# chenxing1999/recsys-benchmark

Hardware: NVIDIA B200
Metric: DeepFM train samples/s (Criteo shape) (higher is better)
Workload: dtype f32

## Files before the change

include/rsb.h:

```cpp
#ifndef RSB_H_
#define RSB_H_

#include <stdint.h>

#if defined(__GNUC__)
#define RSB_API __attribute__((visibility("default")))
#else
#define RSB_API
#endif

#ifdef __cplusplus
extern "C" {
#endif

typedef enum {
  RSB_OK = 0,
  RSB_ERR_BAD_ARG = 10001,
  RSB_ERR_UNSUPPORTED = 10002,
  RSB_ERR_WORKSPACE = 10003
} rsb_status;

typedef enum {
  RSB_KIND_VANILLA = 0,
  RSB_KIND_QR_MULT = 1,
  RSB_KIND_QR_ADD = 2,
  RSB_KIND_QR_CAT = 3,
  RSB_KIND_PEP = 4,
  RSB_KIND_MASK = 5,
  RSB_KIND_OPTEMBED = 6
} rsb_kind;

typedef enum {
  RSB_PEP_GLOBAL = 0,
  RSB_PEP_DIMENSION = 1,
  RSB_PEP_FEATURE = 2,
  RSB_PEP_FEATURE_DIM = 3
} rsb_pep_threshold;

typedef enum {
  RSB_APPLY_DENSE = 0,
  RSB_APPLY_SPARSE_ADAM = 1,
  RSB_APPLY_SPARSE_SGD = 2,
  RSB_APPLY_SHARD_ATOMIC = 3
} rsb_apply;

RSB_API const char* rsb_version(void);
RSB_API const char* rsb_error_string(int code);
RSB_API int64_t rsb_launch_count(void);
RSB_API int rsb_row_width_supported(int32_t width);

RSB_API int rsb_lookup_fwd(int32_t kind, const void* idx, int32_t idx_is_i32, const int64_t* offsets,
                   int64_t B, int32_t F, int32_t D,
                   const float* table, int64_t n_rows, int64_t n_global,
                   const float* table1, int64_t divider,
                   const void* aux, int32_t aux_mode, const int64_t* mask_d_idx,
                   const float* fc, const float* bias,
                   float* out_emb, float* out_yfm, float* out_sum, int64_t* out_rows,
                   int32_t* err_flag, float* amax_slots, void* stream);
#define RSB_LOOKUP_AMAX_SLOTS 1024

RSB_API int rsb_lookup_bwd_rows(int32_t kind, const int64_t* rows, int64_t B, int32_t F, int32_t D,
                        const float* table, int64_t n_rows, const float* table1, int64_t divider,
                        const void* aux, int32_t aux_mode, const int64_t* mask_d_idx,
                        const float* emb, const float* S, const float* g_yfm, const float* g_deep,
                        float* rg_main, float* rg_aux, float* fc_grad, void* stream);

RSB_API int rsb_fc_grad(const int64_t* rows, const float* g_yfm, int64_t B, int32_t F, float* fc_grad, void* stream);

RSB_API int rsb_fc_grad_sorted(const uint32_t* sorted_keys, const uint32_t* perm, int64_t n, const float* g_yfm, int32_t F,
                               float* fc_grad, void* workspace, int64_t workspace_bytes, void* stream);

RSB_API int64_t rsb_qr_bwd_fused_workspace_bytes(int64_t B, int32_t D);
RSB_API int rsb_qr_bwd_fused(int32_t kind, const int64_t* rows, int64_t B, int32_t F, int32_t D,
                             const float* table, int64_t n_rows, const float* table1, int64_t divider,
                             const float* emb, const float* S, const float* g_yfm, const float* g_deep,
                             float* rg_main, float* table1_grad, float* fc_grad, void* workspace,
                             int64_t workspace_bytes, void* stream);

RSB_API int64_t rsb_sort_workspace_bytes(int64_t n);
RSB_API int rsb_sort_rows(const int64_t* keys, int64_t n, int64_t n_rows, int64_t key_div, int64_t key_mod,
                  uint32_t* sorted_keys, uint32_t* perm, void* workspace, int64_t workspace_bytes,
                  void* stream);

RSB_API int64_t rsb_segment_workspace_bytes(int64_t n, int32_t E);
RSB_API int rsb_segment_reduce_apply(int32_t apply, const uint32_t* sorted_keys, const uint32_t* perm, int64_t n,
                             const float* row_grads, int32_t E,
                             float* dst, float* exp_avg, float* exp_avg_sq,
                             float lr, float beta1, float beta2, float eps, int64_t step,
                             void* workspace, int64_t workspace_bytes, void* stream);

RSB_API int64_t rsb_small_table_workspace_bytes(int64_t n_rows, int32_t E);
RSB_API int rsb_small_table_grad(const int64_t* keys, int64_t n, int64_t key_div, int64_t key_mod,
                         const float* row_grads, int32_t E, int64_t n_rows, float* dst,
                         void* workspace, int64_t workspace_bytes, void* stream);

RSB_API int rsb_pep_threshold_table(const float* weight, const float* s, int32_t threshold_type, int64_t n_rows,
                            int32_t D, float* out, int64_t* count, void* stream);
RSB_API int rsb_pep_dense_bwd(const float* weight, const float* s, int32_t threshold_type, int64_t n_rows, int32_t D,
                      const float* g_table, float* g_weight, float* g_s_full, void* stream);
RSB_API int rsb_optembed_eval_weight(const float* weight, const float* t_row, const int64_t* mask_d_row, int32_t norm,
                             int64_t n_rows, int32_t D, float* out, int64_t* count, void* stream);
RSB_API int rsb_mask_table(const float* weight, const uint8_t* mask, int64_t numel, float* out, void* stream);
RSB_API int rsb_sigmoid(const float* s, int64_t numel, float* out, void* stream);

RSB_API int rsb_csr_lookup_fwd(const void* idx, int32_t idx_is_i32, const int64_t* offsets, int64_t B, int32_t F,
                               int32_t D, const float* values, const void* crow, int32_t crow_bytes, const void* col,
                               int32_t col_bytes, int64_t n_rows, const float* fc, const float* bias, float* out_emb,
                               float* out_yfm, int32_t* err_flag, void* stream);

RSB_API int rsb_dhe_encode(const void* ids, int32_t ids_is_i32, int64_t n, int64_t prefix, const int64_t* slopes,
                           const int64_t* bias, const int64_t* primes, int32_t k, int64_t m, int32_t small_operands,
                           float* out, void* stream);

typedef enum { RSB_PLANES_BF16X3 = 0, RSB_PLANES_FP16X2 = 1 } rsb_planes_format_id;
typedef struct {
  int32_t format;
  int32_t max_scale_exp;
  float* amax;
} rsb_planes_format;

typedef struct {
  const void* planes;
  int64_t rows, cols, ld, plane_stride;
  int32_t mn_major;
  int64_t batch_row_step, batch_col_step;
  rsb_planes_format fmt;
} rsb_planes_operand;

typedef enum {
  RSB_EPI_LINEAR = 0,
  RSB_EPI_RELU_DROPOUT_PLANES = 1,
  RSB_EPI_MASK_PLANES = 2,
  RSB_EPI_MASK_F32 = 3
} rsb_epilogue_mode;

typedef struct {
  int32_t mode;
  void* out_planes;
  int64_t out_ld, out_plane_stride;
  int32_t ones_col;
  uint8_t* mask;
  float p;
  float* d_amax;
  float* bn_partials;
} rsb_gemm_epilogue;

RSB_API int rsb_relu_dropout_planes(const float* x, int64_t M, int32_t N, int64_t ldx, float p, uint64_t seed, uint64_t offset,
                                    const uint64_t* offset_dev, int32_t ones_col, void* out_planes, int64_t out_ld,
                                    int64_t plane_stride, uint8_t* mask, void* stream);
RSB_API int rsb_dropout_keep_mask(uint8_t* mask, int64_t numel, float p, uint64_t seed, uint64_t offset,
                                  const uint64_t* offset_dev, void* stream);

RSB_API int rsb_split_planes(const float* in, int64_t rows, int64_t cols, int64_t ld, int32_t transpose, int32_t ones_col,
                             void* out_planes, int64_t out_ld, int64_t plane_stride, const rsb_planes_format* fmt ,
                             void* stream);
RSB_API int rsb_rank1_absmax(const float* g_row, int64_t M, const float* w_col, int64_t N, float mul, float* amax_out,
                             void* stream);
RSB_API int rsb_absmax(const float* in, int64_t rows, int64_t cols, int64_t ld, float* amax_out, void* stream);
RSB_API int rsb_rank1_mask_planes(const float* g_row, const float* w_col, const uint8_t* mask, int64_t M, int32_t N, float p,
                                  void* out_planes, int64_t out_ld, int64_t plane_stride, void* stream);
RSB_API int64_t rsb_gemm_planes_workspace_bytes(int64_t M, int64_t N, int64_t K, int64_t batch, int32_t split_k);
RSB_API int rsb_gemm_planes(const rsb_planes_operand* A, const rsb_planes_operand* B, int64_t M, int64_t N, int64_t K,
                            int64_t batch, int32_t split_k, const float* C, float* D, int64_t ldd, int64_t d_batch_stride,
                            const float* bias, float alpha, float beta, const rsb_gemm_epilogue* epilogue ,
                            void* workspace, int64_t workspace_bytes, void* stream);

RSB_API int64_t rsb_bn_workspace_bytes(int64_t M, int32_t N);
RSB_API int rsb_bn_train_fwd_stats(const float* z, int64_t M, int32_t N, int64_t ldz, const float* gamma, const float* beta,
                                   float eps, float momentum, float* running_mean, float* running_var, float* stats,
                                   float* affine, float bound_mul, float* act_amax, void* workspace, int64_t workspace_bytes,
                                   void* stream);
RSB_API int64_t rsb_gemm_bn_partials_bytes(int64_t M, int64_t N, int64_t K, int32_t format);
RSB_API int rsb_bn_finalize_partials(const float* parts, int64_t M, int32_t N, const float* gamma, const float* beta, float eps,
                                     float momentum, float* running_mean, float* running_var, float* stats, float* affine,
                                     float bound_mul, float* act_amax, void* workspace, int64_t workspace_bytes, void* stream);
RSB_API int rsb_bn_relu_dropout_planes(const float* z, int64_t M, int32_t N, int64_t ldz, const float* affine, float p,
                                       uint64_t seed, uint64_t offset, const uint64_t* offset_dev, int32_t ones_col,
                                       void* out_planes, int64_t out_ld, int64_t plane_stride, uint8_t* mask,
                                       const rsb_planes_format* fmt , void* stream);
RSB_API int rsb_bn_train_bwd_planes(const float* g, const float* z, int64_t M, int32_t N, int64_t ldg, int64_t ldz,
                                    const float* stats, const float* gamma, float* sums, void* out_planes, int64_t out_ld,
                                    int64_t plane_stride, const rsb_planes_format* fmt ,
                                    const float* g_amax , void* workspace,
                                    int64_t workspace_bytes, void* stream);

RSB_API int rsb_relu_dropout_fwd(const float* x, int64_t numel, float p, uint64_t seed, uint64_t offset,
                                 const uint64_t* offset_dev , float* y,
                                 uint8_t* mask, void* stream);
RSB_API int rsb_relu_dropout_bwd(const float* g, const uint8_t* mask, int64_t M, int32_t N, float p, float* gx,
                                 float* colsum, void* workspace, int64_t workspace_bytes, void* stream);
RSB_API int64_t rsb_colsum_workspace_bytes(int64_t M, int32_t N);
RSB_API int rsb_colsum(const float* x, int64_t M, int32_t N, int64_t ld, float* out, void* workspace,
                       int64_t workspace_bytes, void* stream);
RSB_API int rsb_relu_dropout_dot_fwd(const float* x, int64_t M, int32_t N, float p, uint64_t seed, uint64_t offset,
                                     const uint64_t* offset_dev, const float* w, const float* bias, const float* affine,
                                     float* y, uint8_t* mask, float* out, void* stream);
RSB_API int rsb_relu_dropout_bwd_rank1(const float* g_row, const float* w_col, const uint8_t* mask, int64_t M, int32_t N,
                                       float p, float* gx, float* colsum, void* workspace, int64_t workspace_bytes,
                                       void* stream);
RSB_API int rsb_colsum_weighted(const float* x, const float* row_weight, int64_t M, int32_t N, int64_t ld, float* out,
                                void* workspace, int64_t workspace_bytes, void* stream);

RSB_API int rsb_dcn_gate_mix_fwd(const float* p2, const float* xl, const float* gates, int64_t B, int32_t Dm,
                                 int32_t E, int32_t r, float* h2, float* g, float* g2, void* stream);
RSB_API int rsb_dcn_cross_out_fwd(const float* t0, const float* x0, const float* xl, const float* bias,
                                  const float* g, int64_t B, int32_t Dm, int32_t E, float* x_next, void* stream);
RSB_API int rsb_dcn_cross_out_bwd(const float* g_next, const float* x0, const float* t0, const float* bias,
                                  const float* g, int64_t B, int32_t Dm, int32_t E, float* gT, float* gx0,
                                  float* dsg, void* stream);
RSB_API int rsb_dcn_gate_mix_bwd(const float* g_g2, const float* h2, const float* g, const float* dsg,
                                 const float* gates, const float* g_next, int64_t B, int32_t Dm, int32_t E,
                                 int32_t r, float* g_p2, float* dg, float* g_xl, void* stream);

#define RSB_IPC_HANDLE_BYTES 64
RSB_API int rsb_shared_alloc(int64_t bytes, void** dev_ptr_out );
RSB_API int rsb_shared_free(void* dev_ptr);
RSB_API int rsb_ipc_get_handle(const void* dev_ptr, uint8_t* h_handle );
RSB_API int rsb_ipc_open_handle(const uint8_t* h_handle , void** dev_ptr_out );
RSB_API int rsb_ipc_close_handle(void* dev_ptr);
RSB_API int rsb_lookup_fwd_sharded(const void* idx, int32_t idx_is_i32, const int64_t* offsets, int64_t B, int32_t F,
                                   int32_t D, const float* const* table_shards, const float* fc_replicated,
                                   int32_t G, int64_t n_global, const float* bias, const float* hot_table,
                                   const int64_t* hot_map, float* out_emb, float* out_yfm,
                                   float* out_sum, int64_t* out_rows, int32_t* err_flag, float* amax_slots ,
                                   void* stream);
RSB_API int rsb_lookup_fwd_sharded_kind(int32_t kind, const void* idx, int32_t idx_is_i32, const int64_t* offsets, int64_t B,
                                        int32_t F, int32_t D, const float* const* table_shards, int32_t G, int64_t n_rows,
                                        int64_t n_global, const float* table1, int64_t divider, const void* aux,
                                        const void* const* aux_shards, int32_t aux_mode, const int64_t* mask_d_idx,
                                        const float* fc_replicated, const float* bias, float* out_emb, float* out_yfm,
                                        float* out_sum, int64_t* out_rows, int32_t* err_flag, float* amax_slots, void* stream);
RSB_API int rsb_lookup_bwd_rows_sharded(int32_t kind, const int64_t* rows, int64_t B, int32_t F, int32_t D,
                                        const float* const* table_shards, int32_t G, int64_t n_rows, const float* table1,
                                        int64_t divider, const void* aux, const void* const* aux_shards, int32_t aux_mode,
                                        const int64_t* mask_d_idx, const float* emb, const float* S, const float* g_yfm,
                                        const float* g_deep, float* rg_main, float* rg_aux, void* stream);
RSB_API int rsb_segment_scatter_shards(const uint32_t* sorted_keys, const uint32_t* perm, int64_t n,
                                       const float* row_grads, int32_t E, float* const* grad_shards, int32_t G,
                                       float scale, const int64_t* hot_map, int32_t n_fields, float* hot_grad,
                                       void* workspace, int64_t workspace_bytes, void* stream);

RSB_API int rsb_records_unpack(const void* records, int64_t B, int32_t F, int32_t* ids_out, float* labels_out, void* stream);

#define RSB_ADAM_CHUNK 4096
#define RSB_ADAM_MAX_TENSORS 64
typedef struct {
  float* param;
  const float* grad;
  float* exp_avg;
  float* exp_avg_sq;
  int64_t numel;
} rsb_adam_tensor;
RSB_API int rsb_adam_dense(const rsb_adam_tensor* h_tensors, int32_t n_tensors, const int32_t* block_map, int64_t n_blocks,
                           double lr, double beta1, double beta2, double eps, double weight_decay, int64_t step, void* stream);

#ifdef __cplusplus
}
#endif
#endif
```

recsys-benchmark_b200/_lib.py:

```python
from __future__ import annotations

import ctypes as C
import os
from typing import Optional

import torch

_PKG = os.path.dirname(os.path.abspath(__file__))
LIB_PATH = os.path.join(_PKG, "librsb.so")

KIND_VANILLA, KIND_QR_MULT, KIND_QR_ADD, KIND_QR_CAT, KIND_PEP, KIND_MASK, KIND_OPTEMBED = range(7)
PEP_GLOBAL, PEP_DIMENSION, PEP_FEATURE, PEP_FEATURE_DIM = range(4)
APPLY_DENSE, APPLY_SPARSE_ADAM, APPLY_SPARSE_SGD, APPLY_SHARD_ATOMIC = range(4)

PEP_TYPES = {"global": PEP_GLOBAL, "dimension": PEP_DIMENSION, "feature": PEP_FEATURE,
             "feature_dim": PEP_FEATURE_DIM}
QR_KINDS = {"mult": KIND_QR_MULT, "add": KIND_QR_ADD, "cat": KIND_QR_CAT}

_p, _i32, _i64, _f = C.c_void_p, C.c_int32, C.c_int64, C.c_float

class PlanesFormat(C.Structure):

    _fields_ = [("format", C.c_int32), ("max_scale_exp", C.c_int32), ("amax", C.c_void_p)]


PLANES_BF16X3, PLANES_FP16X2 = 0, 1


class PlanesOperand(C.Structure):

    _fields_ = [("planes", C.c_void_p), ("rows", C.c_int64), ("cols", C.c_int64), ("ld", C.c_int64),
                ("plane_stride", C.c_int64), ("mn_major", C.c_int32), ("batch_row_step", C.c_int64),
                ("batch_col_step", C.c_int64), ("fmt", PlanesFormat)]


class GemmEpilogue(C.Structure):

    _fields_ = [("mode", C.c_int32), ("out_planes", C.c_void_p), ("out_ld", C.c_int64), ("out_plane_stride", C.c_int64),
                ("ones_col", C.c_int32), ("mask", C.c_void_p), ("p", C.c_float), ("d_amax", C.c_void_p),
                ("bn_partials", C.c_void_p)]


EPI_LINEAR, EPI_RELU_DROPOUT_PLANES, EPI_MASK_PLANES, EPI_MASK_F32 = range(4)

PROTOTYPES = {
    "rsb_version": (C.c_char_p, []),
    "rsb_error_string": (C.c_char_p, [C.c_int]),
    "rsb_launch_count": (_i64, []),
    "rsb_row_width_supported": (C.c_int, [_i32]),
    "rsb_lookup_fwd": (C.c_int, [_i32, _p, _i32, _p, _i64, _i32, _i32, _p, _i64, _i64, _p, _i64, _p, _i32, _p,
                                 _p, _p, _p, _p, _p, _p, _p, _p, _p]),
    "rsb_lookup_bwd_rows": (C.c_int, [_i32, _p, _i64, _i32, _i32, _p, _i64, _p, _i64, _p, _i32, _p, _p, _p, _p, _p,
                                      _p, _p, _p, _p]),
    "rsb_fc_grad": (C.c_int, [_p, _p, _i64, _i32, _p, _p]),
    "rsb_fc_grad_sorted": (C.c_int, [_p, _p, _i64, _p, _i32, _p, _p, _i64, _p]),
    "rsb_qr_bwd_fused_workspace_bytes": (_i64, [_i64, _i32]),
    "rsb_qr_bwd_fused": (C.c_int, [_i32, _p, _i64, _i32, _i32, _p, _i64, _p, _i64, _p, _p, _p, _p, _p, _p, _p, _p,
                                   _i64, _p]),
    "rsb_sort_workspace_bytes": (_i64, [_i64]),
    "rsb_sort_rows": (C.c_int, [_p, _i64, _i64, _i64, _i64, _p, _p, _p, _i64, _p]),
    "rsb_segment_workspace_bytes": (_i64, [_i64, _i32]),
    "rsb_segment_reduce_apply": (C.c_int, [_i32, _p, _p, _i64, _p, _i32, _p, _p, _p, _f, _f, _f, _f, _i64, _p,
                                           _i64, _p]),
    "rsb_small_table_workspace_bytes": (_i64, [_i64, _i32]),
    "rsb_small_table_grad": (C.c_int, [_p, _i64, _i64, _i64, _p, _i32, _i64, _p, _p, _i64, _p]),
    "rsb_pep_threshold_table": (C.c_int, [_p, _p, _i32, _i64, _i32, _p, _p, _p]),
    "rsb_pep_dense_bwd": (C.c_int, [_p, _p, _i32, _i64, _i32, _p, _p, _p, _p]),
    "rsb_optembed_eval_weight": (C.c_int, [_p, _p, _p, _i32, _i64, _i32, _p, _p, _p]),
    "rsb_mask_table": (C.c_int, [_p, _p, _i64, _p, _p]),
    "rsb_sigmoid": (C.c_int, [_p, _i64, _p, _p]),
    "rsb_csr_lookup_fwd": (C.c_int, [_p, _i32, _p, _i64, _i32, _i32, _p, _p, _i32, _p, _i32, _i64, _p, _p, _p, _p,
                                     _p, _p]),
    "rsb_dhe_encode": (C.c_int, [_p, _i32, _i64, _i64, _p, _p, _p, _i32, _i64, _i32, _p, _p]),
    "rsb_split_planes": (C.c_int, [_p, _i64, _i64, _i64, _i32, _i32, _p, _i64, _i64, C.POINTER(PlanesFormat), _p]),
    "rsb_absmax": (C.c_int, [_p, _i64, _i64, _i64, _p, _p]),
    "rsb_rank1_absmax": (C.c_int, [_p, _i64, _p, _i64, _f, _p, _p]),
    "rsb_relu_dropout_planes": (C.c_int, [_p, _i64, _i32, _i64, _f, C.c_uint64, C.c_uint64, _p, _i32, _p, _i64, _i64, _p, _p]),
    "rsb_dropout_keep_mask": (C.c_int, [_p, _i64, _f, C.c_uint64, C.c_uint64, _p, _p]),
    "rsb_rank1_mask_planes": (C.c_int, [_p, _p, _p, _i64, _i32, _f, _p, _i64, _i64, _p]),
    "rsb_gemm_planes_workspace_bytes": (_i64, [_i64, _i64, _i64, _i64, _i32]),
    "rsb_gemm_planes": (C.c_int, [C.POINTER(PlanesOperand), C.POINTER(PlanesOperand), _i64, _i64, _i64, _i64, _i32, _p,
                                  _p, _i64, _i64, _p, _f, _f, C.POINTER(GemmEpilogue), _p, _i64, _p]),
    "rsb_relu_dropout_fwd": (C.c_int, [_p, _i64, _f, C.c_uint64, C.c_uint64, _p, _p, _p, _p]),
    "rsb_relu_dropout_bwd": (C.c_int, [_p, _p, _i64, _i32, _f, _p, _p, _p, _i64, _p]),
    "rsb_colsum_workspace_bytes": (_i64, [_i64, _i32]),
    "rsb_colsum": (C.c_int, [_p, _i64, _i32, _i64, _p, _p, _i64, _p]),
    "rsb_relu_dropout_dot_fwd": (C.c_int, [_p, _i64, _i32, _f, C.c_uint64, C.c_uint64, _p, _p, _p, _p, _p, _p, _p, _p]),
    "rsb_bn_workspace_bytes": (_i64, [_i64, _i32]),
    "rsb_gemm_bn_partials_bytes": (_i64, [_i64, _i64, _i64, _i32]),
    "rsb_bn_finalize_partials": (C.c_int, [_p, _i64, _i32, _p, _p, _f, _f, _p, _p, _p, _p, _f, _p, _p, _i64, _p]),
    "rsb_bn_train_fwd_stats": (C.c_int, [_p, _i64, _i32, _i64, _p, _p, _f, _f, _p, _p, _p, _p, _f, _p, _p, _i64, _p]),
    "rsb_bn_relu_dropout_planes": (C.c_int, [_p, _i64, _i32, _i64, _p, _f, C.c_uint64, C.c_uint64, _p, _i32, _p, _i64, _i64,
                                             _p, C.POINTER(PlanesFormat), _p]),
    "rsb_bn_train_bwd_planes": (C.c_int, [_p, _p, _i64, _i32, _i64, _i64, _p, _p, _p, _p, _i64, _i64,
                                          C.POINTER(PlanesFormat), _p, _p, _i64, _p]),
    "rsb_relu_dropout_bwd_rank1": (C.c_int, [_p, _p, _p, _i64, _i32, _f, _p, _p, _p, _i64, _p]),
    "rsb_colsum_weighted": (C.c_int, [_p, _p, _i64, _i32, _i64, _p, _p, _i64, _p]),
    "rsb_dcn_gate_mix_fwd": (C.c_int, [_p, _p, _p, _i64, _i32, _i32, _i32, _p, _p, _p, _p]),
    "rsb_dcn_cross_out_fwd": (C.c_int, [_p, _p, _p, _p, _p, _i64, _i32, _i32, _p, _p]),
    "rsb_dcn_cross_out_bwd": (C.c_int, [_p, _p, _p, _p, _p, _i64, _i32, _i32, _p, _p, _p, _p]),
    "rsb_dcn_gate_mix_bwd": (C.c_int, [_p, _p, _p, _p, _p, _p, _i64, _i32, _i32, _i32, _p, _p, _p, _p]),
    "rsb_shared_alloc": (C.c_int, [_i64, C.POINTER(C.c_void_p)]),
    "rsb_shared_free": (C.c_int, [_p]),
    "rsb_ipc_get_handle": (C.c_int, [_p, C.c_char_p]),
    "rsb_ipc_open_handle": (C.c_int, [C.c_char_p, C.POINTER(C.c_void_p)]),
    "rsb_ipc_close_handle": (C.c_int, [_p]),
    "rsb_lookup_fwd_sharded": (C.c_int, [_p, _i32, _p, _i64, _i32, _i32, _p, _p, _i32, _i64, _p, _p, _p, _p, _p, _p,
                                         _p, _p, _p, _p]),
    "rsb_records_unpack": (C.c_int, [_p, _i64, _i32, _p, _p, _p]),
    "rsb_adam_dense": (C.c_int, [_p, _i32, _p, _i64, C.c_double, C.c_double, C.c_double, C.c_double, C.c_double, _i64, _p]),
    "rsb_lookup_fwd_sharded_kind": (C.c_int, [_i32, _p, _i32, _p, _i64, _i32, _i32, _p, _i32, _i64, _i64, _p, _i64, _p, _p,
                                              _i32, _p, _p, _p, _p, _p, _p, _p, _p, _p, _p]),
    "rsb_lookup_bwd_rows_sharded": (C.c_int, [_i32, _p, _i64, _i32, _i32, _p, _i32, _i64, _p, _i64, _p, _p, _i32, _p, _p,
                                              _p, _p, _p, _p, _p, _p]),
    "rsb_segment_scatter_shards": (C.c_int, [_p, _p, _i64, _p, _i32, _p, _i32, _f, _p, _i32, _p, _p, _i64, _p]),
}
LOOKUP_AMAX_SLOTS = 1024
ADAM_CHUNK = 4096
ADAM_MAX_TENSORS = 64


class AdamTensor(C.Structure):

    _fields_ = [("param", C.c_void_p), ("grad", C.c_void_p), ("exp_avg", C.c_void_p), ("exp_avg_sq", C.c_void_p),
                ("numel", C.c_int64)]

_lib: Optional[C.CDLL] = None


def load() -> C.CDLL:
    global _lib
    if _lib is not None:
        return _lib
    if not os.path.exists(LIB_PATH):
        raise RuntimeError(
            f"rsb: {LIB_PATH} not found. Build it with `python recsys-benchmark_b200/build.py` "
            "(or __graft_entry__.build()). There is no CPU / PyTorch fallback for the hot path.")
    lib = C.CDLL(LIB_PATH)
    for name, (res, args) in PROTOTYPES.items():
        fn = getattr(lib, name)
        fn.restype = res
        fn.argtypes = args
    _lib = lib
    return lib


def version() -> str:
    return load().rsb_version().decode()


def check(rc: int, what: str = "") -> None:
    if rc != 0:
        msg = load().rsb_error_string(int(rc)).decode()
        raise RuntimeError(f"rsb {what} failed (code {rc}): {msg}")


def ptr(t: Optional[torch.Tensor]) -> Optional[int]:
    if t is None:
        return None
    return t.data_ptr()


_raw_stream = getattr(torch._C, "_cuda_getCurrentRawStream", None)


def stream_ptr(device=None) -> int:
    if _raw_stream is not None and type(device) is torch.device and device.index is not None:
        return _raw_stream(device.index)
    return torch.cuda.current_stream(device).cuda_stream


def require_cuda(*tensors) -> torch.device:
    dev = None
    for t in tensors:
        if t is None:
            continue
        if not t.is_cuda:
            raise RuntimeError("rsb: the hot path runs on CUDA tensors only (no CPU fallback); "
                               "move the module and its inputs to a B200 device")
        if dev is None:
            dev = t.device
        elif t.device != dev:
            raise RuntimeError(f"rsb: tensors on different devices ({dev} vs {t.device})")
    return dev
```

recsys-benchmark_b200/csrc/batchnorm.cu:

```cuda
#include <cuda_bf16.h>

#include "common.cuh"

namespace rsb {

constexpr int kBnThreads = 128;

template <int MODE>
__global__ void __launch_bounds__(kBnThreads) bn_slab_sums_kernel(const float* __restrict__ z, const float* __restrict__ g,
                                                                  long long M, int N, long long ldz, long long ldg,
                                                                  const float* __restrict__ mean,
                                                                  const float* __restrict__ rstd,
                                                                  float* __restrict__ partials) {
  const int n4 = N / 4;
  const long long rows_per = (M + gridDim.x - 1) / gridDim.x;
  const long long r0 = rows_per * blockIdx.x;
  long long r1 = r0 + rows_per;
  if (r1 > M) r1 = M;
  for (int c4 = threadIdx.x; c4 < n4; c4 += kBnThreads) {
    float4 k, rs = make_float4(1.f, 1.f, 1.f, 1.f);
    if (MODE == 0) {
      k = __ldg(reinterpret_cast<const float4*>(z) + c4);
    } else {
      k = __ldg(reinterpret_cast<const float4*>(mean) + c4);
      rs = __ldg(reinterpret_cast<const float4*>(rstd) + c4);
    }
    float4 sa = make_float4(0.f, 0.f, 0.f, 0.f), sb = sa;
    long long r = r0;
    constexpr int U = MODE == 0 ? 8 : 4;
    for (; r + U <= r1; r += U) {
      float4 zv[U], gv[U];
#pragma unroll
      for (int u = 0; u < U; ++u) {
        zv[u] = __ldg(reinterpret_cast<const float4*>(z + (r + u) * ldz) + c4);
        if (MODE == 1) gv[u] = __ldg(reinterpret_cast<const float4*>(g + (r + u) * ldg) + c4);
      }
#pragma unroll
      for (int u = 0; u < U; ++u) {
        const float4 d = make_float4(zv[u].x - k.x, zv[u].y - k.y, zv[u].z - k.z, zv[u].w - k.w);
        if (MODE == 0) {
          sa.x += d.x; sa.y += d.y; sa.z += d.z; sa.w += d.w;
          sb.x = fmaf(d.x, d.x, sb.x); sb.y = fmaf(d.y, d.y, sb.y); sb.z = fmaf(d.z, d.z, sb.z); sb.w = fmaf(d.w, d.w, sb.w);
        } else {
          sa.x += gv[u].x; sa.y += gv[u].y; sa.z += gv[u].z; sa.w += gv[u].w;
          sb.x = fmaf(gv[u].x, d.x * rs.x, sb.x); sb.y = fmaf(gv[u].y, d.y * rs.y, sb.y);
          sb.z = fmaf(gv[u].z, d.z * rs.z, sb.z); sb.w = fmaf(gv[u].w, d.w * rs.w, sb.w);
        }
      }
    }
    for (; r < r1; ++r) {
      const float4 zv = __ldg(reinterpret_cast<const float4*>(z + r * ldz) + c4);
      const float4 d = make_float4(zv.x - k.x, zv.y - k.y, zv.z - k.z, zv.w - k.w);
      if (MODE == 0) {
        sa.x += d.x; sa.y += d.y; sa.z += d.z; sa.w += d.w;
        sb.x = fmaf(d.x, d.x, sb.x); sb.y = fmaf(d.y, d.y, sb.y); sb.z = fmaf(d.z, d.z, sb.z); sb.w = fmaf(d.w, d.w, sb.w);
      } else {
        const float4 gv = __ldg(reinterpret_cast<const float4*>(g + r * ldg) + c4);
        sa.x += gv.x; sa.y += gv.y; sa.z += gv.z; sa.w += gv.w;
        sb.x = fmaf(gv.x, d.x * rs.x, sb.x); sb.y = fmaf(gv.y, d.y * rs.y, sb.y);
        sb.z = fmaf(gv.z, d.z * rs.z, sb.z); sb.w = fmaf(gv.w, d.w * rs.w, sb.w);
      }
    }
    float* pa = partials + ((long long)blockIdx.x * 2) * N;
    reinterpret_cast<float4*>(pa)[c4] = sa;
    reinterpret_cast<float4*>(pa + N)[c4] = sb;
  }
}

template <int MODE>
__global__ void __launch_bounds__(1024) bn_finalize_kernel(const float* __restrict__ partials, int nblk, int N, long long M,
                                                          const float* __restrict__ z_row0, const float* __restrict__ gamma,
                                                          const float* __restrict__ beta, float eps, float momentum,
                                                          float* __restrict__ running_mean, float* __restrict__ running_var,
                                                          float* __restrict__ stats, float* __restrict__ affine,
                                                          const float* __restrict__ fwd_stats, float bound_mul,
                                                          const float* __restrict__ g_amax, float* __restrict__ amax) {
  __shared__ double red_a[32][33], red_b[32][33];
  const int tx = threadIdx.x & 31, ty = threadIdx.x >> 5;
  const int c = blockIdx.x * 32 + tx;
  float fa = 0.f, fb = 0.f, ca = 0.f, cb = 0.f;
  if (c < N) {
#pragma unroll 4
    for (int b = ty; b < nblk; b += 32) {
      const float va = __ldg(partials + ((long long)b * 2) * N + c) - ca;
      const float vb = __ldg(partials + ((long long)b * 2 + 1) * N + c) - cb;
      const float ta = __fadd_rn(fa, va), tb = __fadd_rn(fb, vb);
      ca = __fsub_rn(__fsub_rn(ta, fa), va);
      cb = __fsub_rn(__fsub_rn(tb, fb), vb);
      fa = ta;
      fb = tb;
    }
  }
  red_a[ty][tx] = (double)fa - (double)ca;
  red_b[ty][tx] = (double)fb - (double)cb;
  __syncthreads();
  if (ty != 0 || c >= N) return;
  double sa = 0.0, sb = 0.0;
#pragma unroll
  for (int y = 0; y < 32; ++y) {
    sa += red_a[y][tx];
    sb += red_b[y][tx];
  }
  if (MODE == 0) {
    const double m = (double)M;
    const double dm = sa / m;
    double var = sb / m - dm * dm;
    if (var < 0.0) var = 0.0;
    const float mean = (float)((double)__ldg(z_row0 + c) + dm);
    const float rstd = (float)(1.0 / sqrt(var + (double)eps));
    stats[c] = mean;
    stats[N + c] = rstd;
    const float ga = gamma ? __ldg(gamma + c) : 1.f, be = beta ? __ldg(beta + c) : 0.f;
    const float sc = ga * rstd;
    affine[c] = sc;
    affine[N + c] = be - mean * sc;
    if (running_mean) running_mean[c] = (1.f - momentum) * running_mean[c] + momentum * mean;
    if (running_var) {
      const float unbiased = (float)(var * (m / (m > 1.0 ? m - 1.0 : 1.0)));
      running_var[c] = (1.f - momentum) * running_var[c] + momentum * unbiased;
    }
    if (amax) {
      const float bound = bound_mul * (fabsf(ga) * sqrtf((float)M) * 1.001f + fabsf(be));
      if (bound > 0.f && bound < 3.0e38f) atomic_max_nonneg(amax, bound);
    }
  } else {
    stats[c] = (float)sa;
    stats[N + c] = (float)sb;
    if (amax) {
      const float rs = __ldg(fwd_stats + N + c), ga = gamma ? __ldg(gamma + c) : 1.f;
      const float bound = fabsf(ga * rs) * __ldg(g_amax) * (2.f + sqrtf((float)M)) * 1.001f;
      if (bound > 0.f && bound < 3.0e38f) atomic_max_nonneg(amax, bound);
    }
  }
}

__global__ void __launch_bounds__(1024) bn_parts_fold_kernel(const float* __restrict__ parts, long long groups, int N, long long M,
                                                             float* __restrict__ out) {
  __shared__ float red_a[32][33], red_b[32][33];
  const int tx = threadIdx.x & 31, ty = threadIdx.x >> 5;
  const int c = blockIdx.x * 32 + tx;
  const long long per = (groups + gridDim.y - 1) / gridDim.y;
  const long long g0 = per * blockIdx.y;
  long long g1 = g0 + per;
  if (g1 > groups) g1 = groups;
  float t1 = 0.f, t2 = 0.f;
  if (c < N) {
    const float k0 = __ldg(parts + 2 * (long long)N + c);
#pragma unroll 4
    for (long long g = g0 + ty; g < g1; g += 32) {
      long long n = M - g * 32;
      n = n > 32 ? 32 : n;
      if (n <= 0) break;
      const float* pg = parts + g * 3 * (long long)N;
      const float s1 = __ldg(pg + c), s2 = __ldg(pg + (long long)N + c), d = __ldg(pg + 2 * (long long)N + c) - k0;
      const float nd = (float)n * d;
      t1 += nd + s1;
      t2 += fmaf(d, 2.f * s1 + nd, s2);
    }
  }
  red_a[ty][tx] = t1;
  red_b[ty][tx] = t2;
  __syncthreads();
  if (ty != 0 || c >= N) return;
  t1 = 0.f;
  t2 = 0.f;
#pragma unroll
  for (int y = 0; y < 32; ++y) {
    t1 += red_a[y][tx];
    t2 += red_b[y][tx];
  }
  out[((long long)blockIdx.y * 2) * N + c] = t1;
  out[((long long)blockIdx.y * 2 + 1) * N + c] = t2;
}

__global__ void __launch_bounds__(256) bn_apply_planes_kernel(const float* __restrict__ z, long long M, int N, long long ldz,
                                                              const float* __restrict__ affine, float drop_scale,
                                                              unsigned thr, unsigned long long seed, unsigned long long offset,
                                                              const unsigned long long* __restrict__ offset_dev,
                                                              uint16_t* __restrict__ out, long long out_ld,
                                                              long long plane_stride, unsigned char* __restrict__ mask,
                                                              int ones_col, PlaneFmt fmt, FastDiv row_div) {
  Philox rng{(unsigned)seed, (unsigned)(seed >> 32)};
  if (offset_dev) offset += *offset_dev;
  const float ps = fmt.scale();
  const int n4 = N / 4;
  const int n4o = (N + 7) / 8 * 2 + (ones_col ? 2 : 0);
  const long long total = M * n4o;
  const bool small = total < (1ll << 32);
  for (long long i = (long long)blockIdx.x * blockDim.x + threadIdx.x; i < total; i += (long long)gridDim.x * blockDim.x) {
    const long long r = small ? (long long)fastdiv((unsigned)i, row_div) : i / n4o;
    const int c4 = (int)(i - r * n4o);
    float4 v = make_float4(0.f, 0.f, 0.f, 0.f);
    if (c4 < n4) {
      const float4 zv = __ldg(reinterpret_cast<const float4*>(z + r * ldz) + c4);
      const float4 sc = __ldg(reinterpret_cast<const float4*>(affine) + c4);
      const float4 sh = __ldg(reinterpret_cast<const float4*>(affine + N) + c4);
      const float4 y = make_float4(fmaf(zv.x, sc.x, sh.x), fmaf(zv.y, sc.y, sh.y), fmaf(zv.z, sc.z, sh.z), fmaf(zv.w, sc.w, sh.w));
      uint4 q = make_uint4(0xffffffffu, 0xffffffffu, 0xffffffffu, 0xffffffffu);
      if (thr) q = rng(offset + (unsigned long long)(r * n4 + c4));
      uchar4 m;
      m.x = (y.x > 0.f) && (q.x >= thr); m.y = (y.y > 0.f) && (q.y >= thr);
      m.z = (y.z > 0.f) && (q.z >= thr); m.w = (y.w > 0.f) && (q.w >= thr);
      *reinterpret_cast<uchar4*>(mask + r * (long long)N + c4 * 4) = m;
      v = make_float4(m.x ? y.x * drop_scale : 0.f, m.y ? y.y * drop_scale : 0.f, m.z ? y.z * drop_scale : 0.f,
                      m.w ? y.w * drop_scale : 0.f);
    } else if (ones_col && c4 * 4 == ((N + 7) & ~7)) {
      v.x = 1.f;
    }
    const float vv[4] = {v.x, v.y, v.z, v.w};
    store_planes<4>(out + r * out_ld + c4 * 4, plane_stride, vv, fmt.format, ps);
  }
}

__global__ void __launch_bounds__(256) bn_bwd_planes_kernel(const float* __restrict__ g, const float* __restrict__ z,
                                                            long long M, int N, long long ldg, long long ldz,
                                                            const float* __restrict__ stats, const float* __restrict__ sums,
                                                            const float* __restrict__ gamma, uint16_t* __restrict__ out,
                                                            long long out_ld, long long plane_stride, PlaneFmt fmt,
                                                            FastDiv row_div) {
  const float ps = fmt.scale();
  const int n4 = N / 4;
  const int n4o = (N + 7) / 8 * 2;
  const float inv_m = 1.0f / (float)M;
  const long long total = M * n4o;
  const bool small = total < (1ll << 32);
  for (long long i = (long long)blockIdx.x * blockDim.x + threadIdx.x; i < total; i += (long long)gridDim.x * blockDim.x) {
    const long long r = small ? (long long)fastdiv((unsigned)i, row_div) : i / n4o;
    const int c4 = (int)(i - r * n4o);
    float4 v = make_float4(0.f, 0.f, 0.f, 0.f);
    if (c4 < n4) {
      const float4 gv = __ldg(reinterpret_cast<const float4*>(g + r * ldg) + c4);
      const float4 zv = __ldg(reinterpret_cast<const float4*>(z + r * ldz) + c4);
      const float4 mu = __ldg(reinterpret_cast<const float4*>(stats) + c4);
      const float4 rs = __ldg(reinterpret_cast<const float4*>(stats + N) + c4);
      const float4 db = __ldg(reinterpret_cast<const float4*>(sums) + c4);
      const float4 dg = __ldg(reinterpret_cast<const float4*>(sums + N) + c4);
      const float4 ga = gamma ? __ldg(reinterpret_cast<const float4*>(gamma) + c4) : make_float4(1.f, 1.f, 1.f, 1.f);
#define RSB_BN_BWD(f) (ga.f * rs.f * (gv.f - db.f * inv_m - (zv.f - mu.f) * rs.f * dg.f * inv_m))
      v = make_float4(RSB_BN_BWD(x), RSB_BN_BWD(y), RSB_BN_BWD(z), RSB_BN_BWD(w));
#undef RSB_BN_BWD
    }
    const float vv[4] = {v.x, v.y, v.z, v.w};
    store_planes<4>(out + r * out_ld + c4 * 4, plane_stride, vv, fmt.format, ps);
  }
}

static int bn_blocks(long long M, int per_sm = 8) {
  long long b = (long long)sm_count() * per_sm;
  const long long need = (M + 31) / 32;
  if (b > need) b = need;
  return b < 1 ? 1 : (int)b;
}

}

using namespace rsb;

extern "C" RSB_API int64_t rsb_bn_workspace_bytes(int64_t M, int32_t N) {
  if (M <= 0 || N <= 0) return 256;
  return (int64_t)bn_blocks(M) * 2 * N * 4 + 256;
}

extern "C" RSB_API int rsb_bn_train_fwd_stats(const float* z, int64_t M, int32_t N, int64_t ldz, const float* gamma,
                                              const float* beta, float eps, float momentum, float* running_mean,
                                              float* running_var, float* stats, float* affine, float bound_mul,
                                              float* act_amax, void* workspace, int64_t workspace_bytes, void* stream) {
  if (!z || !stats || !affine || M <= 0 || N <= 0) return RSB_ERR_BAD_ARG;
  if (N % 4 || ldz % 4 || !aligned16(z) || !aligned16(stats) || !aligned16(affine) || (gamma && !aligned16(gamma)) ||
      (beta && !aligned16(beta)))
    return RSB_ERR_UNSUPPORTED;
  if (!workspace || workspace_bytes < rsb_bn_workspace_bytes(M, N)) return RSB_ERR_WORKSPACE;
  float* partials = reinterpret_cast<float*>((reinterpret_cast<uintptr_t>(workspace) + 255) / 256 * 256);
  cudaStream_t st = reinterpret_cast<cudaStream_t>(stream);
  const int nblk = bn_blocks(M);
  bn_slab_sums_kernel<0><<<nblk, kBnThreads, 0, st>>>(z, nullptr, M, N, ldz, 0, nullptr, nullptr, partials);
  RSB_CHECK_LAUNCH();
  bn_finalize_kernel<0><<<(N + 31) / 32, 1024, 0, st>>>(partials, nblk, N, M, z, gamma, beta, eps, momentum, running_mean,
                                                     running_var, stats, affine, nullptr, bound_mul, nullptr, act_amax);
  RSB_CHECK_LAUNCH();
  note_launch(2);
  return RSB_OK;
}

constexpr int kBnPartSlices = 16;

extern "C" RSB_API int rsb_bn_finalize_partials(const float* parts, int64_t M, int32_t N, const float* gamma, const float* beta,
                                                float eps, float momentum, float* running_mean, float* running_var, float* stats,
                                                float* affine, float bound_mul, float* act_amax, void* workspace,
                                                int64_t workspace_bytes, void* stream) {
  if (!parts || !stats || !affine || M <= 0 || N <= 0) return RSB_ERR_BAD_ARG;
  if (!workspace || workspace_bytes < (int64_t)kBnPartSlices * 2 * N * 4 + 256) return RSB_ERR_WORKSPACE;
  float* sl = reinterpret_cast<float*>((reinterpret_cast<uintptr_t>(workspace) + 255) / 256 * 256);
  cudaStream_t st = reinterpret_cast<cudaStream_t>(stream);
  const long long groups = (M + 127) / 128 * 4;
  int slices = kBnPartSlices;
  if (slices > groups) slices = (int)groups;
  bn_parts_fold_kernel<<<dim3((N + 31) / 32, slices), 1024, 0, st>>>(parts, groups, N, M, sl);
  RSB_CHECK_LAUNCH();
  bn_finalize_kernel<0><<<(N + 31) / 32, 1024, 0, st>>>(sl, slices, N, M, parts + 2 * (long long)N, gamma, beta, eps, momentum,
                                                     running_mean, running_var, stats, affine, nullptr, bound_mul, nullptr, act_amax);
  RSB_CHECK_LAUNCH();
  note_launch(2);
  return RSB_OK;
}

extern "C" RSB_API int rsb_bn_relu_dropout_planes(const float* z, int64_t M, int32_t N, int64_t ldz, const float* affine, float p,
                                                  uint64_t seed, uint64_t offset, const uint64_t* offset_dev, int32_t ones_col,
                                                  void* out_planes, int64_t out_ld, int64_t plane_stride, uint8_t* mask,
                                                  const rsb_planes_format* fmt, void* stream) {
  if (!z || !affine || !out_planes || !mask || M < 0 || N <= 0 || p < 0.f || p >= 1.f || !plane_fmt_ok(fmt)) return RSB_ERR_BAD_ARG;
  if (M == 0) return RSB_OK;
  if (N % 4 || ldz % 4 || out_ld % 8 || plane_stride % 8 || out_ld < ((N + 7) / 8) * 8 + (ones_col ? 8 : 0) || !aligned16(z) ||
      !aligned16(affine) || !aligned16(out_planes) || (reinterpret_cast<uintptr_t>(mask) & 3u))
    return RSB_ERR_UNSUPPORTED;
  const long long total = M * ((N + 7) / 8 * 2 + (ones_col ? 2 : 0));
  long long blocks = (total + 255) / 256;
  const long long cap = (long long)sm_count() * 16;
  if (blocks > cap) blocks = cap;
  bn_apply_planes_kernel<<<(unsigned)blocks, 256, 0, reinterpret_cast<cudaStream_t>(stream)>>>(
      z, M, N, ldz, affine, 1.0f / (1.0f - p), (unsigned)(p * 4294967296.0), seed, offset,
      reinterpret_cast<const unsigned long long*>(offset_dev), reinterpret_cast<uint16_t*>(out_planes), out_ld, plane_stride,
      mask, ones_col, plane_fmt(fmt), make_fastdiv((unsigned long long)((N + 7) / 8 * 2 + (ones_col ? 2 : 0))));
  RSB_CHECK_LAUNCH();
  note_launch(1);
  return RSB_OK;
}

extern "C" RSB_API int rsb_bn_train_bwd_planes(const float* g, const float* z, int64_t M, int32_t N, int64_t ldg, int64_t ldz,
                                               const float* stats, const float* gamma, float* sums, void* out_planes,
                                               int64_t out_ld, int64_t plane_stride, const rsb_planes_format* fmt,
                                               const float* g_amax, void* workspace, int64_t workspace_bytes, void* stream) {
  if (!g || !z || !stats || !sums || !out_planes || M <= 0 || N <= 0 || !plane_fmt_ok(fmt)) return RSB_ERR_BAD_ARG;
  if (fmt && fmt->format == kPlanesFp16x2 && !g_amax) return RSB_ERR_BAD_ARG;
  if (N % 4 || ldg % 4 || ldz % 4 || out_ld % 8 || plane_stride % 8 || out_ld < ((N + 7) / 8) * 8 || !aligned16(g) ||
      !aligned16(z) || !aligned16(stats) || !aligned16(sums) || !aligned16(out_planes) || (gamma && !aligned16(gamma)))
    return RSB_ERR_UNSUPPORTED;
  if (!workspace || workspace_bytes < rsb_bn_workspace_bytes(M, N)) return RSB_ERR_WORKSPACE;
  float* partials = reinterpret_cast<float*>((reinterpret_cast<uintptr_t>(workspace) + 255) / 256 * 256);
  cudaStream_t st = reinterpret_cast<cudaStream_t>(stream);
  const int nblk = bn_blocks(M, 4);
  const bool h = fmt && fmt->format == kPlanesFp16x2;
  bn_slab_sums_kernel<1><<<nblk, kBnThreads, 0, st>>>(z, g, M, N, ldz, ldg, stats, stats + N, partials);
  RSB_CHECK_LAUNCH();
  bn_finalize_kernel<1><<<(N + 31) / 32, 1024, 0, st>>>(partials, nblk, N, M, nullptr, gamma, nullptr, 0.f, 0.f, nullptr, nullptr,
                                                     sums, nullptr, stats, 1.f, h ? g_amax : nullptr, h ? fmt->amax : nullptr);
  RSB_CHECK_LAUNCH();
  const long long total = M * ((N + 7) / 8 * 2);
  long long blocks = (total + 255) / 256;
  const long long cap = (long long)sm_count() * 16;
  if (blocks > cap) blocks = cap;
  bn_bwd_planes_kernel<<<(unsigned)blocks, 256, 0, st>>>(g, z, M, N, ldg, ldz, stats, sums, gamma,
                                                         reinterpret_cast<uint16_t*>(out_planes), out_ld, plane_stride,
                                                         plane_fmt(fmt), make_fastdiv((unsigned long long)((N + 7) / 8 * 2)));
  RSB_CHECK_LAUNCH();
  note_launch(3);
  return RSB_OK;
}
```

recsys-benchmark_b200/linalg.py:

```python
from __future__ import annotations

from typing import Optional

import torch

from . import _lib as L
from . import functional as RF
from . import planes as P

MIN_FLOPS = 1 << 22


def _aligned(*tensors) -> bool:
    return all(t is None or t.data_ptr() % 16 == 0 for t in tensors)


def gemm_supported(m: int, n: int, k: int, lda: int, ldb: int, ldd: int, trans_a: bool, trans_b: bool) -> bool:
    if trans_a and trans_b:
        return False
    return min(m, n, k) > 0 and n % 4 == 0 and ldd % 4 == 0


def weight_planes(w: torch.Tensor, transpose: bool = False, fmt: int = P.BF16X3) -> P.Planes:
    attr = ("_rsb_planes_t" if transpose else "_rsb_planes") + ("_h" if fmt == P.FP16X2 else "")
    cached = getattr(w, attr, None)
    key = (w._version, w.data_ptr(), tuple(w.shape))
    if cached is not None and cached[0] == key:
        return cached[1]
    w2 = w.detach().reshape(-1, w.shape[-1])
    amax = None
    if fmt == P.FP16X2:
        other = getattr(w, ("_rsb_planes_h" if transpose else "_rsb_planes_t_h"), None)
        amax = other[1].amax if (other is not None and other[0] == key) else P.absmax(w2)
    pl = P.split(w2, transpose=transpose, fmt=fmt, amax=amax)
    setattr(w, attr, (key, pl))
    return pl


MLP_PLANES_FORMAT = P.FP16X2
BN_STATS_IN_GEMM = False


def gemm(a: torch.Tensor, b: torch.Tensor, trans_a: bool = False, trans_b: bool = False,
         bias: Optional[torch.Tensor] = None, out: Optional[torch.Tensor] = None, alpha: float = 1.0,
         beta: float = 0.0, c: Optional[torch.Tensor] = None, split_k: int = 1,
         a_planes: Optional[P.Planes] = None, b_planes: Optional[P.Planes] = None) -> torch.Tensor:
    dev = L.require_cuda(a, b, bias, c)
    assert a.dim() == 2 and b.dim() == 2 and a.dtype == torch.float32 and b.dtype == torch.float32
    k, m = (a.shape if trans_a else a.shape[::-1])
    kb, n = (b.shape[::-1] if trans_b else b.shape)
    assert k == kb, f"inner dimensions differ: {k} vs {kb}"
    if out is None:
        out = torch.empty(m, n, dtype=torch.float32, device=dev)
    if not gemm_supported(m, n, k, 0, 0, out.stride(0), trans_a, trans_b) or out.stride(1) != 1 or \
            not _aligned(bias, c, out):
        raise RuntimeError("rsb gemm: shape not supported by the tensor-core kernel (N and ldd must be multiples of 4)")
    pa = a_planes if a_planes is not None else P.split(a)
    pb = b_planes if b_planes is not None else P.split(b)
    return P.gemm(pa, pb, m, n, k, a_mn_major=trans_a, b_mn_major=not trans_b, bias=bias, out=out, alpha=alpha,
                  beta=beta, c=c, split_k=1 if split_k == 1 else 0)


def _fwd_gemm(xp: P.Planes, weight: torch.Tensor, bias: Optional[torch.Tensor]) -> torch.Tensor:
    n, k = weight.shape
    return P.gemm(xp, weight_planes(weight, fmt=xp.fmt), xp.rows, n, k, bias=bias, split_k=1)


def _dx_gemm(gp: P.Planes, weight: torch.Tensor) -> torch.Tensor:
    n_out, n_in = weight.shape
    return P.gemm(gp, weight_planes(weight, transpose=True, fmt=gp.fmt), gp.rows, n_in, n_out, split_k=1)


def _dw_gemm(gp: P.Planes, xp: P.Planes) -> torch.Tensor:
    return P.gemm(gp, xp, gp.cols, xp.cols, gp.rows, a_mn_major=True, b_mn_major=True, split_k=0)


class _ExpertMatMul(torch.autograd.Function):

    @staticmethod
    def forward(ctx, h, c):
        e, r, r2 = c.shape
        bsz = h.shape[0]
        hp = P.split(h)
        cp = weight_planes(c)
        out = torch.empty(bsz, e * r2, dtype=torch.float32, device=h.device)
        P.gemm(hp, cp, bsz, r2, r, a_mn_major=False, b_mn_major=True, out=out, batch=e, a_steps=(0, r),
               b_steps=(r, 0), d_batch_stride=r2, split_k=1)
        ctx.hp = hp
        ctx.save_for_backward(c)
        ctx.shape = (bsz, e, r, r2)
        return out

    @staticmethod
    def backward(ctx, g):
        (c,) = ctx.saved_tensors
        bsz, e, r, r2 = ctx.shape
        hp, ctx.hp = ctx.hp, None
        gp = P.split(g)
        gh = gc = None
        if ctx.needs_input_grad[0]:
            gh = torch.empty(bsz, e * r, dtype=torch.float32, device=g.device)
            P.gemm(gp, weight_planes(c), bsz, r, r2, a_mn_major=False, b_mn_major=False, out=gh, batch=e,
                   a_steps=(0, r2), b_steps=(r, 0), d_batch_stride=r, split_k=1)
        if ctx.needs_input_grad[1]:
            gc = torch.empty(e, r, r2, dtype=torch.float32, device=g.device)
            P.gemm(hp, gp, r, r2, bsz, a_mn_major=True, b_mn_major=True, out=gc.view(e * r, r2), batch=e,
                   a_steps=(0, r), b_steps=(0, r2), d_batch_stride=r * r2, split_k=0)
        return gh, gc


def expert_matmul(h: torch.Tensor, c: torch.Tensor) -> torch.Tensor:
    e, r, r2 = c.shape
    bsz = h.shape[0]
    if r % 32 == 0 and r2 % 4 == 0 and 2 * bsz * e * r * r2 >= MIN_FLOPS and h.is_cuda and h.dtype == torch.float32:
        return _ExpertMatMul.apply(h, c)
    return torch.bmm(h.view(bsz, e, r).transpose(0, 1), c).transpose(0, 1).reshape(bsz, e * r2)


def colsum(x: torch.Tensor) -> torch.Tensor:
    if x.dim() == 2 and x.is_cuda and x.shape[1] % 4 == 0 and x.stride(1) == 1 and x.stride(0) % 4 == 0 and \
            x.data_ptr() % 16 == 0 and x.shape[0] >= 256:
        lib = L.load()
        m, n = x.shape
        out = torch.empty(n, dtype=torch.float32, device=x.device)
        ws = RF._ws(lib.rsb_colsum_workspace_bytes(m, n), x.device)
        RF._call("colsum", lib.rsb_colsum, L.ptr(x), m, n, x.stride(0), L.ptr(out), L.ptr(ws), ws.numel(),
                 L.stream_ptr(x.device), nbytes=m * n * 4)
        return out
    return x.sum(0)


_DROPOUT_CALLS = 0
_DROPOUT_DEV_COUNTER = None


def use_device_dropout_counter(device) -> torch.Tensor:
    global _DROPOUT_DEV_COUNTER
    _DROPOUT_DEV_COUNTER = torch.zeros(1, dtype=torch.int64, device=device)
    return _DROPOUT_DEV_COUNTER


def advance_dropout_counter():
    if _DROPOUT_DEV_COUNTER is not None:
        _DROPOUT_DEV_COUNTER.add_(1 << 40)


def _dropout_stream(numel: int):
    global _DROPOUT_CALLS
    _DROPOUT_CALLS += 1
    seed = (int(torch.initial_seed()) * 0x9E3779B97F4A7C15 + _DROPOUT_CALLS * 0xD1B54A32D192ED03) & 0xFFFFFFFFFFFFFFFF
    return seed, (_DROPOUT_CALLS * 0x100000000) & 0xFFFFFFFFFFFFFFFF


def _relu_dropout_fwd(x: torch.Tensor, p: float):
    lib = L.load()
    y = torch.empty_like(x)
    mask = torch.empty(x.shape, dtype=torch.uint8, device=x.device)
    seed, off = _dropout_stream(x.numel())
    RF._call("relu_dropout_fwd", lib.rsb_relu_dropout_fwd, L.ptr(x), x.numel(), float(p), seed, off,
             L.ptr(_DROPOUT_DEV_COUNTER), L.ptr(y), L.ptr(mask), L.stream_ptr(x.device), nbytes=x.numel() * 9)
    return y, mask


def _relu_dropout_bwd(g: torch.Tensor, mask: torch.Tensor, p: float, want_colsum: bool):
    lib = L.load()
    m, n = g.shape
    g = g.contiguous()
    gx = torch.empty_like(g)
    cs = torch.empty(n, dtype=torch.float32, device=g.device) if want_colsum else None
    ws = RF._ws(lib.rsb_colsum_workspace_bytes(m, n), g.device) if want_colsum else None
    RF._call("relu_dropout_bwd", lib.rsb_relu_dropout_bwd, L.ptr(g), L.ptr(mask), m, n, float(p), L.ptr(gx), L.ptr(cs),
             L.ptr(ws), ws.numel() if ws is not None else 0, L.stream_ptr(g.device), nbytes=m * n * 9)
    return gx, cs


def _relu_dropout_dot_fwd(x: torch.Tensor, p: float, w: torch.Tensor, bias: Optional[torch.Tensor],
                          affine: Optional[torch.Tensor] = None):
    lib = L.load()
    m, n = x.shape
    y = torch.empty_like(x)
    mask = torch.empty(x.shape, dtype=torch.uint8, device=x.device)
    out = torch.empty(m, dtype=torch.float32, device=x.device)
    seed, off = _dropout_stream(x.numel())
    RF._call("relu_dropout_dot_fwd", lib.rsb_relu_dropout_dot_fwd, L.ptr(x), m, n, float(p), seed, off,
             L.ptr(_DROPOUT_DEV_COUNTER), L.ptr(w), L.ptr(bias), L.ptr(affine), L.ptr(y), L.ptr(mask), L.ptr(out),
             L.stream_ptr(x.device), nbytes=x.numel() * 9 + m * 4)
    return y, mask, out


def _relu_dropout_bwd_rank1(g_row: torch.Tensor, w_col: torch.Tensor, mask: torch.Tensor, p: float, want_colsum: bool):
    lib = L.load()
    m, n = mask.shape
    gx = torch.empty(m, n, dtype=torch.float32, device=mask.device)
    cs = torch.empty(n, dtype=torch.float32, device=mask.device) if want_colsum else None
    ws = RF._ws(lib.rsb_colsum_workspace_bytes(m, n), mask.device) if want_colsum else None
    RF._call("relu_dropout_bwd_rank1", lib.rsb_relu_dropout_bwd_rank1, L.ptr(g_row), L.ptr(w_col), L.ptr(mask), m, n,
             float(p), L.ptr(gx), L.ptr(cs), L.ptr(ws), ws.numel() if ws is not None else 0,
             L.stream_ptr(mask.device), nbytes=m * n * 5 + m * 4)
    return gx, cs


def _colsum_weighted(x: torch.Tensor, row_weight: torch.Tensor) -> torch.Tensor:
    lib = L.load()
    m, n = x.shape
    out = torch.empty(n, dtype=torch.float32, device=x.device)
    ws = RF._ws(lib.rsb_colsum_workspace_bytes(m, n), x.device)
    RF._call("colsum_weighted", lib.rsb_colsum_weighted, L.ptr(x), L.ptr(row_weight), m, n, x.stride(0), L.ptr(out),
             L.ptr(ws), ws.numel(), L.stream_ptr(x.device), nbytes=m * n * 4 + m * 4)
    return out


def _fusable(x: torch.Tensor) -> bool:
    return (x.is_cuda and x.dtype == torch.float32 and x.dim() == 2 and x.is_contiguous() and x.shape[1] % 4 == 0
            and x.shape[1] <= 2048 and x.data_ptr() % 16 == 0)


class _ReluDropout(torch.autograd.Function):

    @staticmethod
    def forward(ctx, x, p):
        y, mask = _relu_dropout_fwd(x, p)
        ctx.save_for_backward(mask)
        ctx.p = p
        return y

    @staticmethod
    def backward(ctx, g):
        (mask,) = ctx.saved_tensors
        gx, _ = _relu_dropout_bwd(g, mask, ctx.p, False)
        return gx, None


def relu_dropout(x: torch.Tensor, p: float, training: bool) -> torch.Tensor:
    if training and 0.0 < p < 1.0 and _fusable(x):
        return _ReluDropout.apply(x, p)
    return torch.nn.functional.dropout(torch.relu(x), p, training)


class _LinearReluDropout(torch.autograd.Function):

    @staticmethod
    def forward(ctx, x, weight, bias, p, side_dw=False):
        xp = P.split(x)
        z = _fwd_gemm(xp, weight, bias)
        y, mask = _relu_dropout_fwd(z, p)
        ctx.xp = xp
        ctx.save_for_backward(weight, mask)
        ctx.p = p
        ctx.has_bias = bias is not None
        ctx.side_dw = side_dw
        return y

    @staticmethod
    def backward(ctx, gy):
        weight, mask = ctx.saved_tensors
        xp, ctx.xp = ctx.xp, None
        gz, gb = _relu_dropout_bwd(gy, mask, ctx.p, ctx.has_bias and ctx.needs_input_grad[2])
        gp = P.split(gz)
        gx = _dx_gemm(gp, weight) if ctx.needs_input_grad[0] else None
        gw = None
        if ctx.needs_input_grad[1]:
            if ctx.side_dw and gx is not None and _side_dw_safe(weight):
                gw = _dw_on_side_stream(gp, xp)
            else:
                gw = _dw_gemm(gp, xp)
        return gx, gw, gb, None, None


def _has_hooks(weight: torch.Tensor) -> bool:
    return bool(getattr(weight, "_backward_hooks", None)) or bool(getattr(weight, "_post_accumulate_grad_hooks", None))


def _side_dw_safe(weight: torch.Tensor) -> bool:
    return weight.grad is None and not _has_hooks(weight) and not torch.cuda.is_current_stream_capturing()


def _dw_on_side_stream(gp: P.Planes, xp: P.Planes) -> torch.Tensor:
    dev = gp.data.device
    main = torch.cuda.current_stream(dev)
    side = RF.side_stream(dev)
    side.wait_stream(main)
    with torch.cuda.stream(side):
        gw = _dw_gemm(gp, xp)
    try:
        torch.autograd.Variable._execution_engine.queue_callback(lambda keep=(gp, xp): main.wait_stream(side))
    except Exception:
        main.wait_stream(side)
    return gw


class _HeadBlock(torch.autograd.Function):

    @staticmethod
    def forward(ctx, x, weight, bias, p, w_out, b_out):
        ctx.xp = None
        if weight is None:
            z = x
        else:
            ctx.xp = P.split(x)
            z = _fwd_gemm(ctx.xp, weight, bias)
        y, mask, out = _relu_dropout_dot_fwd(z, p, w_out.reshape(-1), b_out)
        ctx.save_for_backward(weight, mask, y, w_out)
        ctx.p = p
        ctx.has_bias = bias is not None
        ctx.has_bout = b_out is not None
        return out.unsqueeze(1)

    @staticmethod
    def backward(ctx, g_out):
        weight, mask, y, w_out = ctx.saved_tensors
        xp, ctx.xp = ctx.xp, None
        g = g_out.reshape(-1).contiguous()
        g_wout = _colsum_weighted(y, g).reshape(w_out.shape) if ctx.needs_input_grad[4] else None
        g_bout = g.sum().reshape(1) if ctx.has_bout and ctx.needs_input_grad[5] else None
        want_gb = weight is not None and ctx.has_bias and ctx.needs_input_grad[2]
        gz, gb = _relu_dropout_bwd_rank1(g, w_out.reshape(-1), mask, ctx.p, want_gb)
        if weight is None:
            return gz, None, None, None, g_wout, g_bout
        gp = P.split(gz)
        gx = _dx_gemm(gp, weight) if ctx.needs_input_grad[0] else None
        gw = _dw_gemm(gp, xp) if ctx.needs_input_grad[1] else None
        return gx, gw, gb, None, g_wout, g_bout


def _use_kernel(m, n, k, *tensors) -> bool:
    return (2 * m * n * k >= MIN_FLOPS and n % 4 == 0 and k % 4 == 0 and _aligned(*tensors)
            and all(t is None or (t.is_cuda and t.dtype == torch.float32) for t in tensors))


class _Linear(torch.autograd.Function):

    @staticmethod
    def forward(ctx, x, weight, bias, side_dw=False):
        xp = P.split(x)
        ctx.xp = xp
        ctx.save_for_backward(weight)
        ctx.has_bias = bias is not None
        ctx.side_dw = side_dw
        return _fwd_gemm(xp, weight, bias)

    @staticmethod
    def backward(ctx, gy):
        (weight,) = ctx.saved_tensors
        xp, ctx.xp = ctx.xp, None
        gy = gy.contiguous()
        gp = P.split(gy)
        gx = gw = gb = None
        if ctx.needs_input_grad[0]:
            gx = _dx_gemm(gp, weight)
        if ctx.needs_input_grad[1]:
            if ctx.side_dw and gx is not None and _side_dw_safe(weight):
                gw = _dw_on_side_stream(gp, xp)
            else:
                gw = _dw_gemm(gp, xp)
        if ctx.has_bias and ctx.needs_input_grad[2]:
            gb = colsum(gy)
        return gx, gw, gb, None


def linear(x: torch.Tensor, weight: torch.Tensor, bias: Optional[torch.Tensor] = None,
           side_dw: bool = False) -> torch.Tensor:
    if x.dim() == 2 and _use_kernel(x.shape[0], weight.shape[0], weight.shape[1], x, weight, bias) and \
            x.stride(1) == 1 and x.stride(0) % 4 == 0:
        return _Linear.apply(x, weight, bias, side_dw)
    return torch.nn.functional.linear(x, weight, bias)


class _MatMul(torch.autograd.Function):

    @staticmethod
    def forward(ctx, a, b):
        ap = P.split(a)
        ctx.ap = ap
        ctx.save_for_backward(b)
        m, k = a.shape
        return P.gemm(ap, weight_planes(b), m, b.shape[1], k, b_mn_major=True, split_k=1)

    @staticmethod
    def backward(ctx, gc):
        (b,) = ctx.saved_tensors
        ap, ctx.ap = ctx.ap, None
        gp = P.split(gc.contiguous())
        ga = gb = None
        if ctx.needs_input_grad[0]:
            ga = P.gemm(gp, weight_planes(b), gp.rows, b.shape[0], b.shape[1], split_k=1)
        if ctx.needs_input_grad[1]:
            gb = P.gemm(ap, gp, ap.cols, gp.cols, ap.rows, a_mn_major=True, b_mn_major=True, split_k=0)
        return ga, gb


def matmul(a: torch.Tensor, b: torch.Tensor) -> torch.Tensor:
    if a.dim() == 2 and b.dim() == 2 and a.stride(1) == 1 and b.stride(1) == 1 and a.stride(0) % 4 == 0 and \
            b.stride(0) % 4 == 0 and _use_kernel(a.shape[0], b.shape[1], a.shape[1], a, b):
        return _MatMul.apply(a, b)
    return torch.matmul(a, b)


FUSE_FORWARD_EPILOGUE = False


class _MlpReluDropout(torch.autograd.Function):

    @staticmethod
    def forward(ctx, x, ps, side_dw, *params):
        n_layers = (len(params) - 2) // 2
        ws, bs = params[0:2 * n_layers:2], params[1:2 * n_layers:2]
        w_out, b_out = params[-2], params[-1]
        planes = [P.split(x, ones_col=True)]
        masks = []
        for i in range(n_layers - 1):
            seed, off = _dropout_stream(x.shape[0] * ws[i].shape[0])
            if FUSE_FORWARD_EPILOGUE:
                yp, mask = P.linear_relu_dropout(planes[-1], weight_planes(ws[i]), bs[i], ps[i], seed, off,
                                                 _DROPOUT_DEV_COUNTER, ones_col=True)
            else:
                z = _fwd_gemm(planes[-1], ws[i], bs[i])
                yp, mask = P.relu_dropout_planes(z, ps[i], seed, off, _DROPOUT_DEV_COUNTER, ones_col=True)
            planes.append(yp)
            masks.append(mask)
        z = _fwd_gemm(planes[-1], ws[-1], bs[-1])
        y, mask, out = _relu_dropout_dot_fwd(z, ps[-1], w_out.reshape(-1), b_out)
        masks.append(mask)
        ctx.planes, ctx.masks, ctx.ps, ctx.side_dw, ctx.n_layers = planes, masks, ps, side_dw, n_layers
        ctx.save_for_backward(y, *params)
        return out.unsqueeze(1)

    @staticmethod
    def backward(ctx, g_out):
        y, *params = ctx.saved_tensors
        n_layers, ps, planes, masks = ctx.n_layers, ctx.ps, ctx.planes, ctx.masks
        ctx.planes = ctx.masks = None
        ws, bs = params[0:2 * n_layers:2], params[1:2 * n_layers:2]
        w_out, b_out = params[-2], params[-1]
        need = ctx.needs_input_grad
        g = g_out.reshape(-1).contiguous()
        grads = [None] * len(params)
        if need[3 + 2 * n_layers]:
            grads[-2] = _colsum_weighted(y, g).reshape(w_out.shape)
        if b_out is not None and need[4 + 2 * n_layers]:
            grads[-1] = g.sum().reshape(1)
        gp = P.rank1_mask_planes(g, w_out.reshape(-1), masks[-1], ps[-1])
        gx = None
        for i in reversed(range(n_layers)):
            gp_prev = None
            if i > 0:
                gp_prev = P.dx_masked(gp, weight_planes(ws[i], transpose=True), masks[i - 1], ps[i - 1])
            elif need[0]:
                gx = _dx_gemm(gp, ws[0])
            want_w, want_b = need[3 + 2 * i], bs[i] is not None and need[4 + 2 * i]
            if want_w or want_b:
                if i == 0 and ctx.side_dw and gx is not None and _side_dw_safe(ws[0]) and \
                        (bs[0] is None or _side_dw_safe(bs[0])):
                    dw, db = _on_side_stream(lambda gp=gp, xp=planes[0]: P.gemm_dw(gp, xp, want_b), (gp, planes[0]))
                else:
                    dw, db = P.gemm_dw(gp, planes[i], want_b)
                grads[2 * i] = dw if want_w else None
                grads[2 * i + 1] = db if want_b else None
            gp = gp_prev
        return (gx, None, None, *grads)


class _MlpBatchNorm(torch.autograd.Function):

    @staticmethod
    def forward(ctx, x, ps, side_dw, bns, x_amax_slots, *params):
        n_layers = (len(params) - 2) // 4
        ws, bs = params[0:4 * n_layers:4], params[1:4 * n_layers:4]
        gammas, betas = params[2:4 * n_layers:4], params[3:4 * n_layers:4]
        w_out, b_out = params[-2], params[-1]
        fmt = MLP_PLANES_FORMAT
        amaxs = torch.zeros(n_layers, 1, dtype=torch.float32, device=x.device) if fmt == P.FP16X2 else None
        x_amax = None
        if amaxs is not None:
            x_amax = P.absmax(x_amax_slots.view(1, -1) if x_amax_slots is not None else x, amaxs[0])
        planes = [P.split(x, ones_col=True, fmt=fmt, amax=x_amax)]
        masks, zs, stats = [], [], []
        y = out = None
        for i in range(n_layers):
            bn = bns[i]
            act_amax = amaxs[i + 1] if (amaxs is not None and i < n_layers - 1) else None
            z, st, affine = P.gemm_bn_stats(planes[-1], weight_planes(ws[i], fmt=planes[-1].fmt), bs[i], gammas[i],
                                            betas[i], bn.eps, bn.momentum,
                                            bn.running_mean if bn.track_running_stats else None,
                                            bn.running_var if bn.track_running_stats else None,
                                            act_amax=act_amax, bound_mul=1.0 / (1.0 - ps[i]), in_epilogue=BN_STATS_IN_GEMM)
            if bn.track_running_stats and bn.num_batches_tracked is not None:
                bn.num_batches_tracked.add_(1)
            if i < n_layers - 1:
                seed, off = _dropout_stream(z.numel())
                yp, mask = P.bn_relu_dropout_planes(z, affine, ps[i], seed, off, _DROPOUT_DEV_COUNTER, ones_col=True,
                                                    fmt=fmt, amax=act_amax)
                planes.append(yp)
            else:
                y, mask, out = _relu_dropout_dot_fwd(z, ps[i], w_out.reshape(-1), b_out, affine)
            masks.append(mask)
            zs.append(z)
            stats.append(st)
        ctx.planes, ctx.masks, ctx.ps, ctx.side_dw, ctx.n_layers = planes, masks, ps, side_dw, n_layers
        ctx.n_z = len(zs)
        ctx.save_for_backward(y, *zs, *stats, *params)
        return out.unsqueeze(1)

    @staticmethod
    def backward(ctx, g_out):
        n_layers, ps, planes, masks = ctx.n_layers, ctx.ps, ctx.planes, ctx.masks
        ctx.planes = ctx.masks = None
        saved = ctx.saved_tensors
        y, zs, stats, params = saved[0], saved[1:1 + n_layers], saved[1 + n_layers:1 + 2 * n_layers], saved[1 + 2 * n_layers:]
        ws, bs = params[0:4 * n_layers:4], params[1:4 * n_layers:4]
        gammas, betas = params[2:4 * n_layers:4], params[3:4 * n_layers:4]
        w_out, b_out = params[-2], params[-1]
        need = ctx.needs_input_grad
        g = g_out.reshape(-1).contiguous()
        grads = [None] * len(params)
        if need[5 + 4 * n_layers]:
            grads[-2] = _colsum_weighted(y, g).reshape(w_out.shape)
        if b_out is not None and need[6 + 4 * n_layers]:
            grads[-1] = g.sum().reshape(1)
        g_r, _ = _relu_dropout_bwd_rank1(g, w_out.reshape(-1), masks[-1], ps[-1], False)
        fmt = planes[0].fmt
        g_amaxs = torch.zeros(n_layers, 1, dtype=torch.float32, device=g.device) if fmt == P.FP16X2 else None
        if g_amaxs is not None:
            P.rank1_absmax(g, w_out.reshape(-1), ps[-1], g_amaxs[n_layers - 1])
        gx = None
        for i in reversed(range(n_layers)):
            gp, d_beta, d_gamma = P.bn_train_bwd_planes(g_r, zs[i], stats[i], gammas[i], fmt=fmt,
                                                        g_amax=g_amaxs[i] if g_amaxs is not None else None)
            if gammas[i] is not None and need[7 + 4 * i]:
                grads[4 * i + 2] = d_gamma
            if betas[i] is not None and need[8 + 4 * i]:
                grads[4 * i + 3] = d_beta
            g_prev = None
            if i > 0:
                g_prev = P.dx_masked(gp, weight_planes(ws[i], transpose=True, fmt=gp.fmt), masks[i - 1], ps[i - 1],
                                     to_planes=False, d_amax=g_amaxs[i - 1] if g_amaxs is not None else None)
            elif need[0]:
                gx = _dx_gemm(gp, ws[0])
            want_w, want_b = need[5 + 4 * i], bs[i] is not None and need[6 + 4 * i]
            if want_w or want_b:
                if i == 0 and ctx.side_dw and gx is not None and _side_dw_safe(ws[0]) and \
                        (bs[0] is None or _side_dw_safe(bs[0])):
                    dw, db = _on_side_stream(lambda gp=gp, xp=planes[0]: P.gemm_dw(gp, xp, want_b), (gp, planes[0]))
                else:
                    dw, db = P.gemm_dw(gp, planes[i], want_b)
                grads[4 * i] = dw if want_w else None
                grads[4 * i + 1] = db if want_b else None
            g_r = g_prev
        return (gx, None, None, None, None, *grads)


def _mlp_batchnorm_pattern(mods, x: torch.Tensor):
    if (len(mods) - 1) % 4 or len(mods) < 5 or not (x.is_cuda and x.dtype == torch.float32 and x.dim() == 2):
        return None
    lins, bns, drops = [], [], []
    width = x.shape[1]
    for j in range(0, len(mods) - 1, 4):
        lin, bn, act, drop = mods[j], mods[j + 1], mods[j + 2], mods[j + 3]
        if not (isinstance(lin, torch.nn.Linear) and isinstance(bn, torch.nn.BatchNorm1d) and
                isinstance(act, torch.nn.ReLU) and isinstance(drop, torch.nn.Dropout)):
            return None
        h = lin.weight.shape[0]
        if lin.weight.shape[1] != width or h % 8 or width % 4 or not 0.0 <= drop.p < 1.0 or h > 2048 or \
                lin.weight.dtype != torch.float32 or not lin.weight.is_cuda or bn.num_features != h or \
                bn.momentum is None or not bn.training or (bn.weight is None) != (bn.bias is None) or \
                (bn.weight is not None and bn.weight.dtype != torch.float32):
            return None
        width = h
        lins.append(lin)
        bns.append(bn)
        drops.append(drop)
    head = mods[-1]
    if not _is_head(head, width) or x.shape[0] < 256:
        return None
    return lins, bns, drops, head


def _on_side_stream(fn, keep):
    dev = torch.cuda.current_device()
    main = torch.cuda.current_stream(dev)
    side = RF.side_stream(dev)
    side.wait_stream(main)
    with torch.cuda.stream(side):
        out = fn()
    try:
        torch.autograd.Variable._execution_engine.queue_callback(lambda keep=keep: main.wait_stream(side))
    except Exception:
        main.wait_stream(side)
    return out


def _mlp_relu_dropout_pattern(mods, x: torch.Tensor):
    if (len(mods) - 1) % 3 or len(mods) < 4 or not (x.is_cuda and x.dtype == torch.float32 and x.dim() == 2):
        return None
    lins, drops = [], []
    width = x.shape[1]
    for j in range(0, len(mods) - 1, 3):
        lin, act, drop = mods[j], mods[j + 1], mods[j + 2]
        if not (isinstance(lin, torch.nn.Linear) and isinstance(act, torch.nn.ReLU) and isinstance(drop, torch.nn.Dropout)):
            return None
        if lin.weight.shape[1] != width or lin.weight.shape[0] % 8 or width % 4 or not 0.0 < drop.p < 1.0 or \
                lin.weight.dtype != torch.float32 or not lin.weight.is_cuda or lin.weight.shape[0] > 2048:
            return None
        width = lin.weight.shape[0]
        lins.append(lin)
        drops.append(drop)
    head = mods[-1]
    if not _is_head(head, width) or x.shape[0] < 256:
        return None
    return lins, drops, head


def _is_head(mod, width: int) -> bool:
    return (isinstance(mod, torch.nn.Linear) and mod.weight.shape[0] == 1 and mod.weight.shape[1] == width
            and width % 4 == 0 and mod.weight.is_cuda and mod.weight.dtype == torch.float32
            and mod.weight.data_ptr() % 16 == 0)


def run_sequential(seq: torch.nn.Sequential, x: torch.Tensor, overlap_first_dw: bool = False,
                   x_amax_slots: Optional[torch.Tensor] = None) -> torch.Tensor:
    mods = list(seq)
    i = 0
    training = seq.training
    if training:
        pat = _mlp_batchnorm_pattern(mods, x)
        if pat is not None:
            lins, bns, drops, head = pat
            params = []
            for lin, bn in zip(lins, bns):
                params += [lin.weight, lin.bias, bn.weight, bn.bias]
            side = overlap_first_dw and not _has_hooks(lins[0].weight) and \
                (lins[0].bias is None or not _has_hooks(lins[0].bias))
            return _MlpBatchNorm.apply(x.contiguous(), tuple(float(d.p) for d in drops), side, tuple(bns), x_amax_slots,
                                       *params, head.weight, head.bias)
        pat = _mlp_relu_dropout_pattern(mods, x)
        if pat is not None:
            lins, drops, head = pat
            params = []
            for lin in lins:
                params += [lin.weight, lin.bias]
            side = overlap_first_dw and not _has_hooks(lins[0].weight) and \
                (lins[0].bias is None or not _has_hooks(lins[0].bias))
            return _MlpReluDropout.apply(x.contiguous(), tuple(float(d.p) for d in drops), side, *params, head.weight,
                                         head.bias)
    while i < len(mods):
        m = mods[i]
        nxt = mods[i + 1] if i + 1 < len(mods) else None
        nx2 = mods[i + 2] if i + 2 < len(mods) else None
        nx3 = mods[i + 3] if i + 3 < len(mods) else None
        if isinstance(m, torch.nn.Linear):
            ok = x.dim() == 2 and x.stride(1) == 1 and x.stride(0) % 4 == 0 and \
                _use_kernel(x.shape[0], m.weight.shape[0], m.weight.shape[1], x, m.weight, m.bias)
            if ok and isinstance(nxt, torch.nn.ReLU) and isinstance(nx2, torch.nn.Dropout) and training and \
                    0.0 < nx2.p < 1.0 and m.weight.shape[0] <= 2048 and _is_head(nx3, m.weight.shape[0]) and \
                    i + 4 == len(mods):
                return _HeadBlock.apply(x, m.weight, m.bias, float(nx2.p), nx3.weight, nx3.bias)
            if ok and isinstance(nxt, torch.nn.ReLU) and isinstance(nx2, torch.nn.Dropout) and training and \
                    0.0 < nx2.p < 1.0 and m.weight.shape[0] <= 2048:
                x = _LinearReluDropout.apply(x, m.weight, m.bias, float(nx2.p),
                                             overlap_first_dw and i == 0 and not _has_hooks(m.weight))
                i += 3
                continue
            x = linear(x, m.weight, m.bias, side_dw=overlap_first_dw and i == 0 and not _has_hooks(m.weight))
            i += 1
            continue
        if isinstance(m, torch.nn.ReLU) and isinstance(nxt, torch.nn.Dropout) and training and 0.0 < nxt.p < 1.0 \
                and i + 3 == len(mods) and _fusable(x) and _is_head(nx2, x.shape[1]) and x.shape[0] >= 256:
            return _HeadBlock.apply(x, None, None, float(nxt.p), nx2.weight, nx2.bias)
        if isinstance(m, torch.nn.ReLU) and isinstance(nxt, torch.nn.Dropout):
            x = relu_dropout(x, float(nxt.p), training)
            i += 2
            continue
        x = m(x)
        i += 1
    return x
```

recsys-benchmark_b200/planes.py:

```python
from __future__ import annotations

import ctypes as C
from typing import Optional

import torch

from . import _lib as L
from . import functional as RF


BF16X3, FP16X2 = L.PLANES_BF16X3, L.PLANES_FP16X2
MAX_SCALE_EXP = 40
ONES_SCALE_EXP = 14


class Planes:

    __slots__ = ("data", "rows", "cols", "fmt", "amax", "max_exp", "_ops")

    def __init__(self, data: torch.Tensor, rows: int, cols: int, fmt: int = BF16X3, amax: Optional[torch.Tensor] = None,
                 max_exp: int = MAX_SCALE_EXP):
        self.data, self.rows, self.cols, self.fmt, self.amax, self.max_exp = data, rows, cols, fmt, amax, max_exp
        self._ops = None

    def format(self) -> L.PlanesFormat:
        return L.PlanesFormat(self.fmt, self.max_exp, self.amax.data_ptr() if self.amax is not None else None)

    def scale(self) -> torch.Tensor:
        if self.fmt != FP16X2:
            return torch.ones((), device=self.data.device)
        a = self.amax.reshape(()).double()
        e = torch.floor(torch.log2(a)) + 1
        se = torch.clamp(14 - e, max=self.max_exp)
        return torch.where(a > 0, torch.exp2(se), torch.ones_like(a)).float()

    @property
    def ld(self) -> int:
        return self.data.shape[2]

    def operand(self, mn_major: bool, row_step: int = 0, col_step: int = 0, cols: Optional[int] = None) -> L.PlanesOperand:
        key = (mn_major, row_step, col_step, cols)
        ops = self._ops
        if ops is None:
            ops = self._ops = {}
        op = ops.get(key)
        if op is None:
            op = ops[key] = L.PlanesOperand(self.data.data_ptr(), self.rows, self.cols if cols is None else cols, self.ld,
                                            self.data.stride(0), int(mn_major), row_step, col_step, self.format())
        return op

    def float(self) -> torch.Tensor:
        x = self.data.double().sum(0)[:, :self.cols]
        return (x / self.scale().double()).float() if self.fmt == FP16X2 else x.float()


def alloc(rows: int, cols: int, device, ones_col: bool = False, fmt: int = BF16X3,
          amax: Optional[torch.Tensor] = None) -> Planes:
    ld = (cols + 7) // 8 * 8 + (8 if ones_col else 0)
    if fmt == FP16X2:
        if amax is None:
            amax = torch.zeros(1, dtype=torch.float32, device=device)
        return Planes(torch.empty(2, rows, ld, dtype=torch.float16, device=device), rows, cols, FP16X2, amax,
                      ONES_SCALE_EXP if ones_col else MAX_SCALE_EXP)
    return Planes(torch.empty(3, rows, ld, dtype=torch.bfloat16, device=device), rows, cols)


def absmax(x: torch.Tensor, out: Optional[torch.Tensor] = None) -> torch.Tensor:
    lib = L.load()
    dev = L.require_cuda(x)
    if out is None:
        out = torch.zeros(1, dtype=torch.float32, device=dev)
    RF._call("absmax", lib.rsb_absmax, L.ptr(x), x.shape[0], x.shape[1], x.stride(0), L.ptr(out), L.stream_ptr(dev),
             nbytes=x.numel() * 4)
    return out


def split(x: torch.Tensor, transpose: bool = False, ones_col: bool = False, fmt: int = BF16X3,
          amax: Optional[torch.Tensor] = None) -> Planes:
    lib = L.load()
    dev = L.require_cuda(x)
    assert x.dim() == 2 and x.dtype == torch.float32
    if x.stride(1) != 1:
        x = x.contiguous()
    rows, cols = x.shape
    orows, ocols = (cols, rows) if transpose else (rows, cols)
    if fmt == FP16X2 and amax is None:
        amax = absmax(x)
    out = alloc(orows, ocols, dev, ones_col, fmt, amax)
    pf = out.format()
    RF._call("split_planes", lib.rsb_split_planes, L.ptr(x), rows, cols, x.stride(0), int(transpose), int(ones_col),
             L.ptr(out.data), out.ld, out.data.stride(0), C.byref(pf), L.stream_ptr(dev),
             nbytes=rows * cols * 4 + out.data.shape[0] * orows * out.ld * 2)
    return out


def _dropout_epilogue(mode: int, out: Optional[Planes], mask: torch.Tensor, p: float, ones_col: bool,
                      d_amax: Optional[torch.Tensor] = None) -> L.GemmEpilogue:
    return L.GemmEpilogue(mode, out.data.data_ptr() if out is not None else None, out.ld if out is not None else 0,
                          out.data.stride(0) if out is not None else 0, int(ones_col), mask.data_ptr(), float(p),
                          d_amax.data_ptr() if d_amax is not None else None)


def dropout_keep_mask(shape, p: float, seed: int, offset: int, offset_dev: Optional[torch.Tensor], device) -> torch.Tensor:
    lib = L.load()
    mask = torch.empty(shape, dtype=torch.uint8, device=device)
    RF._call("dropout_keep_mask", lib.rsb_dropout_keep_mask, L.ptr(mask), mask.numel(), float(p),
             seed & 0xFFFFFFFFFFFFFFFF, offset & 0xFFFFFFFFFFFFFFFF, L.ptr(offset_dev), L.stream_ptr(device),
             nbytes=mask.numel())
    return mask


def gemm(a: Planes, b: Planes, m: int, n: int, k: int, *, a_mn_major: bool = False, b_mn_major: bool = False,
         bias: Optional[torch.Tensor] = None, out: Optional[torch.Tensor] = None, alpha: float = 1.0, beta: float = 0.0,
         c: Optional[torch.Tensor] = None, split_k: int = 0, batch: int = 1, a_steps=(0, 0), b_steps=(0, 0),
         d_batch_stride: int = 0, epilogue: Optional[L.GemmEpilogue] = None, want_out: bool = True,
         b_cols: Optional[int] = None):
    lib = L.load()
    dev = a.data.device
    if out is None and want_out:
        out = torch.empty(m, n, dtype=torch.float32, device=dev)
    nb = lib.rsb_gemm_planes_workspace_bytes(m, n, k, batch, split_k)
    ws = RF._ws(nb, dev)
    oa = a.operand(a_mn_major, *a_steps)
    ob = b.operand(b_mn_major, *b_steps, cols=b_cols)
    kind = ("gemm_planes" if epilogue is None else
            ("gemm_planes", "gemm_planes_relu_dropout", "gemm_planes_masked", "gemm_planes_masked")[epilogue.mode])
    if a_mn_major and b_mn_major:
        kind = "gemm_planes_dw"
    if a.fmt == FP16X2:
        kind += "_h"
    RF._call(kind, lib.rsb_gemm_planes, C.byref(oa), C.byref(ob), m, n, k, batch, split_k, L.ptr(c), L.ptr(out),
             out.stride(0) if out is not None else n, d_batch_stride, L.ptr(bias), alpha, beta,
             C.byref(epilogue) if epilogue is not None else None, L.ptr(ws), ws.numel(), L.stream_ptr(dev),
             nbytes=2 * m * n * k * batch)
    return out


def linear_relu_dropout(xp: Planes, wp: Planes, bias: Optional[torch.Tensor], p: float, seed: int, offset: int,
                        offset_dev: Optional[torch.Tensor] = None, ones_col: bool = True):
    m, n, k = xp.rows, wp.rows, wp.cols
    yp = alloc(m, n, xp.data.device, ones_col)
    mask = dropout_keep_mask((m, n), p, seed, offset, offset_dev, xp.data.device)
    epi = _dropout_epilogue(L.EPI_RELU_DROPOUT_PLANES, yp, mask, p, ones_col)
    gemm(xp, wp, m, n, k, bias=bias, split_k=1, epilogue=epi, want_out=False)
    return yp, mask


def relu_dropout_planes(z: torch.Tensor, p: float, seed: int, offset: int, offset_dev: Optional[torch.Tensor] = None,
                        ones_col: bool = True):
    lib = L.load()
    m, n = z.shape
    yp = alloc(m, n, z.device, ones_col)
    mask = torch.empty(m, n, dtype=torch.uint8, device=z.device)
    RF._call("relu_dropout_planes", lib.rsb_relu_dropout_planes, L.ptr(z), m, n, z.stride(0), float(p),
             seed & 0xFFFFFFFFFFFFFFFF, offset & 0xFFFFFFFFFFFFFFFF, L.ptr(offset_dev), int(ones_col), L.ptr(yp.data), yp.ld,
             yp.data.stride(0), L.ptr(mask), L.stream_ptr(z.device), nbytes=m * n * 5 + 3 * m * yp.ld * 2)
    return yp, mask


def dx_masked(gp: Planes, wtp: Planes, mask: torch.Tensor, p: float, to_planes: bool = True,
              d_amax: Optional[torch.Tensor] = None):
    m, n, k = gp.rows, wtp.rows, wtp.cols
    if to_planes:
        out = alloc(m, n, gp.data.device)
        epi = _dropout_epilogue(L.EPI_MASK_PLANES, out, mask, p, False)
        gemm(gp, wtp, m, n, k, split_k=1, epilogue=epi, want_out=False)
        return out
    epi = _dropout_epilogue(L.EPI_MASK_F32, None, mask, p, False, d_amax)
    return gemm(gp, wtp, m, n, k, split_k=1, epilogue=epi)


def rank1_absmax(g_row: torch.Tensor, w_col: torch.Tensor, p: float, out: Optional[torch.Tensor] = None) -> torch.Tensor:
    lib = L.load()
    dev = g_row.device
    if out is None:
        out = torch.zeros(1, dtype=torch.float32, device=dev)
    RF._call("rank1_absmax", lib.rsb_rank1_absmax, L.ptr(g_row), g_row.numel(), L.ptr(w_col), w_col.numel(),
             1.0 / (1.0 - p), L.ptr(out), L.stream_ptr(dev), nbytes=g_row.numel() * 4)
    return out


def gemm_dw(gp: Planes, xp: Planes, want_bias_grad: bool):
    n_out, n_in, m = gp.cols, xp.cols, gp.rows
    n_pad = (n_in + 7) // 8 * 8
    has_ones = xp.ld >= n_pad + 8
    if want_bias_grad and has_ones:
        full = gemm(gp, xp, n_out, n_pad + 8, m, a_mn_major=True, b_mn_major=True, split_k=0, b_cols=n_pad + 8)
        return full[:, :n_in], full[:, n_pad]
    return gemm(gp, xp, n_out, n_in, m, a_mn_major=True, b_mn_major=True, split_k=0), None


def rank1_mask_planes(g_row: torch.Tensor, w_col: torch.Tensor, mask: torch.Tensor, p: float) -> Planes:
    lib = L.load()
    m, n = mask.shape
    out = alloc(m, n, mask.device)
    RF._call("rank1_mask_planes", lib.rsb_rank1_mask_planes, L.ptr(g_row), L.ptr(w_col), L.ptr(mask), m, n, float(p),
             L.ptr(out.data), out.ld, out.data.stride(0), L.stream_ptr(mask.device), nbytes=m * n * 7 + m * 4)
    return out


def bn_train_stats(z: torch.Tensor, gamma: Optional[torch.Tensor], beta: Optional[torch.Tensor], eps: float,
                   momentum: float, running_mean: Optional[torch.Tensor], running_var: Optional[torch.Tensor],
                   act_amax: Optional[torch.Tensor] = None, bound_mul: float = 1.0):
    lib = L.load()
    m, n = z.shape
    dev = z.device
    stats = torch.empty(2 * n, dtype=torch.float32, device=dev)
    affine = torch.empty(2 * n, dtype=torch.float32, device=dev)
    ws = RF._ws(lib.rsb_bn_workspace_bytes(m, n), dev)
    RF._call("bn_fwd_stats", lib.rsb_bn_train_fwd_stats, L.ptr(z), m, n, z.stride(0), L.ptr(gamma), L.ptr(beta), float(eps),
             float(momentum), L.ptr(running_mean), L.ptr(running_var), L.ptr(stats), L.ptr(affine), float(bound_mul),
             L.ptr(act_amax), L.ptr(ws), ws.numel(), L.stream_ptr(dev), nbytes=m * n * 4)
    return stats, affine


def gemm_bn_stats(xp: Planes, wp: Planes, bias: Optional[torch.Tensor], gamma: Optional[torch.Tensor],
                  beta: Optional[torch.Tensor], eps: float, momentum: float, running_mean: Optional[torch.Tensor],
                  running_var: Optional[torch.Tensor], act_amax: Optional[torch.Tensor] = None, bound_mul: float = 1.0,
                  in_epilogue: bool = True):
    lib = L.load()
    m, n, k = xp.rows, wp.rows, wp.cols
    dev = xp.data.device
    nb = lib.rsb_gemm_bn_partials_bytes(m, n, k, xp.fmt) if in_epilogue else -1
    if nb <= 0:
        z = gemm(xp, wp, m, n, k, bias=bias, split_k=1)
        return (z, *bn_train_stats(z, gamma, beta, eps, momentum, running_mean, running_var, act_amax, bound_mul))
    parts = torch.empty(nb // 4, dtype=torch.float32, device=dev)
    epi = L.GemmEpilogue(L.EPI_LINEAR, None, 0, 0, 0, None, 0.0, None, parts.data_ptr())
    z = gemm(xp, wp, m, n, k, bias=bias, split_k=1, epilogue=epi)
    stats = torch.empty(2 * n, dtype=torch.float32, device=dev)
    affine = torch.empty(2 * n, dtype=torch.float32, device=dev)
    ws = RF._ws(16 * 2 * n * 4 + 512, dev)
    RF._call("bn_finalize_partials", lib.rsb_bn_finalize_partials, L.ptr(parts), m, n, L.ptr(gamma), L.ptr(beta), float(eps),
             float(momentum), L.ptr(running_mean), L.ptr(running_var), L.ptr(stats), L.ptr(affine), float(bound_mul),
             L.ptr(act_amax), L.ptr(ws), ws.numel(), L.stream_ptr(dev), nbytes=parts.numel() * 4)
    return z, stats, affine


def bn_relu_dropout_planes(z: torch.Tensor, affine: torch.Tensor, p: float, seed: int, offset: int,
                           offset_dev: Optional[torch.Tensor] = None, ones_col: bool = True, fmt: int = BF16X3,
                           amax: Optional[torch.Tensor] = None):
    lib = L.load()
    m, n = z.shape
    assert fmt == BF16X3 or amax is not None
    yp = alloc(m, n, z.device, ones_col, fmt, amax)
    pf = yp.format()
    mask = torch.empty(m, n, dtype=torch.uint8, device=z.device)
    RF._call("bn_relu_dropout_planes", lib.rsb_bn_relu_dropout_planes, L.ptr(z), m, n, z.stride(0), L.ptr(affine), float(p),
             seed & 0xFFFFFFFFFFFFFFFF, offset & 0xFFFFFFFFFFFFFFFF, L.ptr(offset_dev), int(ones_col), L.ptr(yp.data), yp.ld,
             yp.data.stride(0), L.ptr(mask), C.byref(pf), L.stream_ptr(z.device),
             nbytes=m * n * 5 + yp.data.shape[0] * m * yp.ld * 2)
    return yp, mask


def bn_train_bwd_planes(g: torch.Tensor, z: torch.Tensor, stats: torch.Tensor, gamma: Optional[torch.Tensor],
                        fmt: int = BF16X3, g_amax: Optional[torch.Tensor] = None):
    lib = L.load()
    m, n = z.shape
    dev = z.device
    sums = torch.empty(2 * n, dtype=torch.float32, device=dev)
    if fmt == FP16X2 and g_amax is None:
        g_amax = absmax(g)
    out = alloc(m, n, dev, fmt=fmt)
    pf = out.format()
    ws = RF._ws(lib.rsb_bn_workspace_bytes(m, n), dev)
    RF._call("bn_bwd_planes", lib.rsb_bn_train_bwd_planes, L.ptr(g), L.ptr(z), m, n, g.stride(0), z.stride(0), L.ptr(stats),
             L.ptr(gamma), L.ptr(sums), L.ptr(out.data), out.ld, out.data.stride(0), C.byref(pf), L.ptr(g_amax), L.ptr(ws),
             ws.numel(), L.stream_ptr(dev), nbytes=m * n * 16 + out.data.shape[0] * m * out.ld * 2)
    return out, sums[:n], sums[n:]
```

Measured before the change: 26.75 million.

## Fuse BN stats, finalize and apply into single cooperative slab kernel

Replaces the separate BN stats reduction, finalize, and apply/relu/dropout/plane-split kernels with a fused cooperative-groups launch over column slabs. The slab is re-read with an L2 keep cache hint, so the second pass should hit L2 instead of HBM. The backward path is restructured the same way. For non-final MLP layers, the forward now runs a plain GEMM followed by this fused BN kernel, replacing the GEMM-epilogue statistics path. This aims to cut launch count and HBM traffic, at the cost of grid-wide synchronisation and dependence on L2 capacity.

```diff
diff --git a/include/rsb.h b/include/rsb.h
--- a/include/rsb.h
+++ b/include/rsb.h
@@ -174,10 +174,12 @@
 RSB_API int rsb_bn_finalize_partials(const float* parts, int64_t M, int32_t N, const float* gamma, const float* beta, float eps,
                                      float momentum, float* running_mean, float* running_var, float* stats, float* affine,
                                      float bound_mul, float* act_amax, void* workspace, int64_t workspace_bytes, void* stream);
-RSB_API int rsb_bn_relu_dropout_planes(const float* z, int64_t M, int32_t N, int64_t ldz, const float* affine, float p,
-                                       uint64_t seed, uint64_t offset, const uint64_t* offset_dev, int32_t ones_col,
-                                       void* out_planes, int64_t out_ld, int64_t plane_stride, uint8_t* mask,
-                                       const rsb_planes_format* fmt , void* stream);
+RSB_API int rsb_bn_train_fwd_planes(const float* z, int64_t M, int32_t N, int64_t ldz, const float* gamma, const float* beta,
+                                    float eps, float momentum, float* running_mean, float* running_var, float* stats,
+                                    float* affine, float bound_mul, float* act_amax, float p, uint64_t seed, uint64_t offset,
+                                    const uint64_t* offset_dev, int32_t ones_col, void* out_planes, int64_t out_ld,
+                                    int64_t plane_stride, uint8_t* mask, const rsb_planes_format* fmt ,
+                                    void* workspace, int64_t workspace_bytes, void* stream);
 RSB_API int rsb_bn_train_bwd_planes(const float* g, const float* z, int64_t M, int32_t N, int64_t ldg, int64_t ldz,
                                     const float* stats, const float* gamma, float* sums, void* out_planes, int64_t out_ld,
                                     int64_t plane_stride, const rsb_planes_format* fmt ,
diff --git a/recsys-benchmark_b200/_lib.py b/recsys-benchmark_b200/_lib.py
--- a/recsys-benchmark_b200/_lib.py
+++ b/recsys-benchmark_b200/_lib.py
@@ -90,8 +90,8 @@
     "rsb_gemm_bn_partials_bytes": (_i64, [_i64, _i64, _i64, _i32]),
     "rsb_bn_finalize_partials": (C.c_int, [_p, _i64, _i32, _p, _p, _f, _f, _p, _p, _p, _p, _f, _p, _p, _i64, _p]),
     "rsb_bn_train_fwd_stats": (C.c_int, [_p, _i64, _i32, _i64, _p, _p, _f, _f, _p, _p, _p, _p, _f, _p, _p, _i64, _p]),
-    "rsb_bn_relu_dropout_planes": (C.c_int, [_p, _i64, _i32, _i64, _p, _f, C.c_uint64, C.c_uint64, _p, _i32, _p, _i64, _i64,
-                                             _p, C.POINTER(PlanesFormat), _p]),
+    "rsb_bn_train_fwd_planes": (C.c_int, [_p, _i64, _i32, _i64, _p, _p, _f, _f, _p, _p, _p, _p, _f, _p, _f, C.c_uint64,
+                                          C.c_uint64, _p, _i32, _p, _i64, _i64, _p, C.POINTER(PlanesFormat), _p, _i64, _p]),
     "rsb_bn_train_bwd_planes": (C.c_int, [_p, _p, _i64, _i32, _i64, _i64, _p, _p, _p, _p, _i64, _i64,
                                           C.POINTER(PlanesFormat), _p, _p, _i64, _p]),
     "rsb_relu_dropout_bwd_rank1": (C.c_int, [_p, _p, _p, _i64, _i32, _f, _p, _p, _p, _i64, _p]),
diff --git a/recsys-benchmark_b200/csrc/batchnorm.cu b/recsys-benchmark_b200/csrc/batchnorm.cu
--- a/recsys-benchmark_b200/csrc/batchnorm.cu
+++ b/recsys-benchmark_b200/csrc/batchnorm.cu
@@ -1,3 +1,4 @@
+#include <cooperative_groups.h>
 #include <cuda_bf16.h>
 
 #include "common.cuh"
@@ -6,131 +7,167 @@
 
 constexpr int kBnThreads = 128;
 
-template <int MODE>
-__global__ void __launch_bounds__(kBnThreads) bn_slab_sums_kernel(const float* __restrict__ z, const float* __restrict__ g,
-                                                                  long long M, int N, long long ldz, long long ldg,
-                                                                  const float* __restrict__ mean,
-                                                                  const float* __restrict__ rstd,
-                                                                  float* __restrict__ partials) {
+struct LdPlain {
+  __device__ __forceinline__ float4 operator()(const float* p) const { return __ldg(reinterpret_cast<const float4*>(p)); }
+};
+struct LdKeep {
+  uint64_t pol;
+  __device__ __forceinline__ float4 operator()(const float* p) const {
+    float4 v;
+    asm("ld.global.nc.L2::cache_hint.v4.f32 {%0, %1, %2, %3}, [%4], %5;"
+        : "=f"(v.x), "=f"(v.y), "=f"(v.z), "=f"(v.w)
+        : "l"(p), "l"(pol));
+    return v;
+  }
+};
+
+template <int MODE, class Ld, int U = MODE == 0 ? 8 : 4>
+__device__ __forceinline__ void bn_row_sums(const float* __restrict__ z, const float* __restrict__ g, long long ldz,
+                                            long long ldg, long long r0, long long r1, int c4, float4 k, float4 rs,
+                                            float4& sa_out, float4& sb_out, Ld ld) {
+  float4 sa = make_float4(0.f, 0.f, 0.f, 0.f), sb = sa;
+  const float* zp = z + r0 * ldz + 4 * c4;
+  const float* gp = MODE == 1 ? g + r0 * ldg + 4 * c4 : nullptr;
+  int n = r1 > r0 ? (int)(r1 - r0) : 0;
+  for (; n >= U; n -= U) {
+    float4 zv[U], gv[U];
+#pragma unroll
+    for (int u = 0; u < U; ++u) {
+      zv[u] = ld(zp + u * ldz);
+      if (MODE == 1) gv[u] = ld(gp + u * ldg);
+    }
+    zp += U * ldz;
+    if (MODE == 1) gp += U * ldg;
+#pragma unroll
+    for (int u = 0; u < U; ++u) {
+      const float4 d = make_float4(zv[u].x - k.x, zv[u].y - k.y, zv[u].z - k.z, zv[u].w - k.w);
+      if (MODE == 0) {
+        sa.x += d.x; sa.y += d.y; sa.z += d.z; sa.w += d.w;
+        sb.x = fmaf(d.x, d.x, sb.x); sb.y = fmaf(d.y, d.y, sb.y); sb.z = fmaf(d.z, d.z, sb.z); sb.w = fmaf(d.w, d.w, sb.w);
+      } else {
+        sa.x += gv[u].x; sa.y += gv[u].y; sa.z += gv[u].z; sa.w += gv[u].w;
+        sb.x = fmaf(gv[u].x, d.x * rs.x, sb.x); sb.y = fmaf(gv[u].y, d.y * rs.y, sb.y);
+        sb.z = fmaf(gv[u].z, d.z * rs.z, sb.z); sb.w = fmaf(gv[u].w, d.w * rs.w, sb.w);
+      }
+    }
+  }
+  for (; n > 0; --n) {
+    const float4 zv = ld(zp);
+    const float4 d = make_float4(zv.x - k.x, zv.y - k.y, zv.z - k.z, zv.w - k.w);
+    zp += ldz;
+    if (MODE == 0) {
+      sa.x += d.x; sa.y += d.y; sa.z += d.z; sa.w += d.w;
+      sb.x = fmaf(d.x, d.x, sb.x); sb.y = fmaf(d.y, d.y, sb.y); sb.z = fmaf(d.z, d.z, sb.z); sb.w = fmaf(d.w, d.w, sb.w);
+    } else {
+      const float4 gv = ld(gp);
+      gp += ldg;
+      sa.x += gv.x; sa.y += gv.y; sa.z += gv.z; sa.w += gv.w;
+      sb.x = fmaf(gv.x, d.x * rs.x, sb.x); sb.y = fmaf(gv.y, d.y * rs.y, sb.y);
+      sb.z = fmaf(gv.z, d.z * rs.z, sb.z); sb.w = fmaf(gv.w, d.w * rs.w, sb.w);
+    }
+  }
+  sa_out = sa;
+  sb_out = sb;
+}
+
+__global__ void __launch_bounds__(kBnThreads) bn_slab_sums_kernel(const float* __restrict__ z, long long M, int N,
+                                                                  long long ldz, float* __restrict__ partials) {
   const int n4 = N / 4;
   const long long rows_per = (M + gridDim.x - 1) / gridDim.x;
   const long long r0 = rows_per * blockIdx.x;
   long long r1 = r0 + rows_per;
   if (r1 > M) r1 = M;
   for (int c4 = threadIdx.x; c4 < n4; c4 += kBnThreads) {
-    float4 k, rs = make_float4(1.f, 1.f, 1.f, 1.f);
-    if (MODE == 0) {
-      k = __ldg(reinterpret_cast<const float4*>(z) + c4);
-    } else {
-      k = __ldg(reinterpret_cast<const float4*>(mean) + c4);
-      rs = __ldg(reinterpret_cast<const float4*>(rstd) + c4);
-    }
-    float4 sa = make_float4(0.f, 0.f, 0.f, 0.f), sb = sa;
-    long long r = r0;
-    constexpr int U = MODE == 0 ? 8 : 4;
-    for (; r + U <= r1; r += U) {
-      float4 zv[U], gv[U];
-#pragma unroll
-      for (int u = 0; u < U; ++u) {
-        zv[u] = __ldg(reinterpret_cast<const float4*>(z + (r + u) * ldz) + c4);
-        if (MODE == 1) gv[u] = __ldg(reinterpret_cast<const float4*>(g + (r + u) * ldg) + c4);
-      }
-#pragma unroll
-      for (int u = 0; u < U; ++u) {
-        const float4 d = make_float4(zv[u].x - k.x, zv[u].y - k.y, zv[u].z - k.z, zv[u].w - k.w);
-        if (MODE == 0) {
-          sa.x += d.x; sa.y += d.y; sa.z += d.z; sa.w += d.w;
-          sb.x = fmaf(d.x, d.x, sb.x); sb.y = fmaf(d.y, d.y, sb.y); sb.z = fmaf(d.z, d.z, sb.z); sb.w = fmaf(d.w, d.w, sb.w);
-        } else {
-          sa.x += gv[u].x; sa.y += gv[u].y; sa.z += gv[u].z; sa.w += gv[u].w;
-          sb.x = fmaf(gv[u].x, d.x * rs.x, sb.x); sb.y = fmaf(gv[u].y, d.y * rs.y, sb.y);
-          sb.z = fmaf(gv[u].z, d.z * rs.z, sb.z); sb.w = fmaf(gv[u].w, d.w * rs.w, sb.w);
-        }
-      }
-    }
-    for (; r < r1; ++r) {
-      const float4 zv = __ldg(reinterpret_cast<const float4*>(z + r * ldz) + c4);
-      const float4 d = make_float4(zv.x - k.x, zv.y - k.y, zv.z - k.z, zv.w - k.w);
-      if (MODE == 0) {
-        sa.x += d.x; sa.y += d.y; sa.z += d.z; sa.w += d.w;
-        sb.x = fmaf(d.x, d.x, sb.x); sb.y = fmaf(d.y, d.y, sb.y); sb.z = fmaf(d.z, d.z, sb.z); sb.w = fmaf(d.w, d.w, sb.w);
-      } else {
-        const float4 gv = __ldg(reinterpret_cast<const float4*>(g + r * ldg) + c4);
-        sa.x += gv.x; sa.y += gv.y; sa.z += gv.z; sa.w += gv.w;
-        sb.x = fmaf(gv.x, d.x * rs.x, sb.x); sb.y = fmaf(gv.y, d.y * rs.y, sb.y);
-        sb.z = fmaf(gv.z, d.z * rs.z, sb.z); sb.w = fmaf(gv.w, d.w * rs.w, sb.w);
-      }
-    }
+    const float4 k = __ldg(reinterpret_cast<const float4*>(z) + c4);
+    float4 sa, sb;
+    bn_row_sums<0>(z, nullptr, ldz, 0, r0, r1, c4, k, k, sa, sb, LdPlain{});
     float* pa = partials + ((long long)blockIdx.x * 2) * N;
     reinterpret_cast<float4*>(pa)[c4] = sa;
     reinterpret_cast<float4*>(pa + N)[c4] = sb;
   }
 }
 
-template <int MODE>
+__device__ __forceinline__ void bn_fold_lane(const float* partials, int nblk, int N, int c, int ty, double& a, double& b) {
+  float fa = 0.f, fb = 0.f, ca = 0.f, cb = 0.f;
+#pragma unroll 4
+  for (int k = ty; k < nblk; k += 32) {
+    const float va = __ldcg(partials + ((long long)k * 2) * N + c) - ca;
+    const float vb = __ldcg(partials + ((long long)k * 2 + 1) * N + c) - cb;
+    const float ta = __fadd_rn(fa, va), tb = __fadd_rn(fb, vb);
+    ca = __fsub_rn(__fsub_rn(ta, fa), va);
+    cb = __fsub_rn(__fsub_rn(tb, fb), vb);
+    fa = ta;
+    fb = tb;
+  }
+  a = (double)fa - (double)ca;
+  b = (double)fb - (double)cb;
+}
+__device__ __forceinline__ void bn_fold_lanes(const double (*red_a)[33], const double (*red_b)[33], int tx, double& sa,
+                                              double& sb) {
+  sa = 0.0;
+  sb = 0.0;
+#pragma unroll
+  for (int y = 0; y < 32; ++y) {
+    sa += red_a[y][tx];
+    sb += red_b[y][tx];
+  }
+}
+
+__device__ __forceinline__ void bn_finish_fwd(int c, int N, long long M, double sa, double sb, const float* z_row0,
+                                              const float* gamma, const float* beta, float eps, float momentum,
+                                              float* running_mean, float* running_var, float* stats, float* affine) {
+  const double m = (double)M;
+  const double dm = sa / m;
+  double var = sb / m - dm * dm;
+  if (var < 0.0) var = 0.0;
+  const float mean = (float)((double)__ldg(z_row0 + c) + dm);
+  const float rstd = (float)(1.0 / sqrt(var + (double)eps));
+  stats[c] = mean;
+  stats[N + c] = rstd;
+  const float ga = gamma ? __ldg(gamma + c) : 1.f, be = beta ? __ldg(beta + c) : 0.f;
+  const float sc = ga * rstd;
+  affine[c] = sc;
+  affine[N + c] = be - mean * sc;
+  if (running_mean) running_mean[c] = (1.f - momentum) * running_mean[c] + momentum * mean;
+  if (running_var) {
+    const float unbiased = (float)(var * (m / (m > 1.0 ? m - 1.0 : 1.0)));
+    running_var[c] = (1.f - momentum) * running_var[c] + momentum * unbiased;
+  }
+}
+
+__device__ __forceinline__ float bn_bound_fwd(int c, long long M, const float* gamma, const float* beta, float bound_mul) {
+  const float ga = gamma ? __ldg(gamma + c) : 1.f, be = beta ? __ldg(beta + c) : 0.f;
+  const float bound = bound_mul * (fabsf(ga) * sqrtf((float)M) * 1.001f + fabsf(be));
+  return bound > 0.f && bound < 3.0e38f ? bound : 0.f;
+}
+__device__ __forceinline__ float bn_bound_bwd(int c, int N, long long M, const float* gamma, const float* fwd_stats,
+                                              const float* g_amax) {
+  const float rs = __ldg(fwd_stats + N + c), ga = gamma ? __ldg(gamma + c) : 1.f;
+  const float bound = fabsf(ga * rs) * *g_amax * (2.f + sqrtf((float)M)) * 1.001f;
+  return bound > 0.f && bound < 3.0e38f ? bound : 0.f;
+}
+
 __global__ void __launch_bounds__(1024) bn_finalize_kernel(const float* __restrict__ partials, int nblk, int N, long long M,
                                                           const float* __restrict__ z_row0, const float* __restrict__ gamma,
                                                           const float* __restrict__ beta, float eps, float momentum,
                                                           float* __restrict__ running_mean, float* __restrict__ running_var,
                                                           float* __restrict__ stats, float* __restrict__ affine,
-                                                          const float* __restrict__ fwd_stats, float bound_mul,
-                                                          const float* __restrict__ g_amax, float* __restrict__ amax) {
+                                                          float bound_mul, float* __restrict__ amax) {
   __shared__ double red_a[32][33], red_b[32][33];
   const int tx = threadIdx.x & 31, ty = threadIdx.x >> 5;
   const int c = blockIdx.x * 32 + tx;
-  float fa = 0.f, fb = 0.f, ca = 0.f, cb = 0.f;
-  if (c < N) {
-#pragma unroll 4
-    for (int b = ty; b < nblk; b += 32) {
-      const float va = __ldg(partials + ((long long)b * 2) * N + c) - ca;
-      const float vb = __ldg(partials + ((long long)b * 2 + 1) * N + c) - cb;
-      const float ta = __fadd_rn(fa, va), tb = __fadd_rn(fb, vb);
-      ca = __fsub_rn(__fsub_rn(ta, fa), va);
-      cb = __fsub_rn(__fsub_rn(tb, fb), vb);
-      fa = ta;
-      fb = tb;
-    }
-  }
-  red_a[ty][tx] = (double)fa - (double)ca;
-  red_b[ty][tx] = (double)fb - (double)cb;
+  double la = 0.0, lb = 0.0;
+  if (c < N) bn_fold_lane(partials, nblk, N, c, ty, la, lb);
+  red_a[ty][tx] = la;
+  red_b[ty][tx] = lb;
   __syncthreads();
   if (ty != 0 || c >= N) return;
-  double sa = 0.0, sb = 0.0;
-#pragma unroll
-  for (int y = 0; y < 32; ++y) {
-    sa += red_a[y][tx];
-    sb += red_b[y][tx];
-  }
-  if (MODE == 0) {
-    const double m = (double)M;
-    const double dm = sa / m;
-    double var = sb / m - dm * dm;
-    if (var < 0.0) var = 0.0;
-    const float mean = (float)((double)__ldg(z_row0 + c) + dm);
-    const float rstd = (float)(1.0 / sqrt(var + (double)eps));
-    stats[c] = mean;
-    stats[N + c] = rstd;
-    const float ga = gamma ? __ldg(gamma + c) : 1.f, be = beta ? __ldg(beta + c) : 0.f;
-    const float sc = ga * rstd;
-    affine[c] = sc;
-    affine[N + c] = be - mean * sc;
-    if (running_mean) running_mean[c] = (1.f - momentum) * running_mean[c] + momentum * mean;
-    if (running_var) {
-      const float unbiased = (float)(var * (m / (m > 1.0 ? m - 1.0 : 1.0)));
-      running_var[c] = (1.f - momentum) * running_var[c] + momentum * unbiased;
-    }
-    if (amax) {
-      const float bound = bound_mul * (fabsf(ga) * sqrtf((float)M) * 1.001f + fabsf(be));
-      if (bound > 0.f && bound < 3.0e38f) atomic_max_nonneg(amax, bound);
-    }
-  } else {
-    stats[c] = (float)sa;
-    stats[N + c] = (float)sb;
-    if (amax) {
-      const float rs = __ldg(fwd_stats + N + c), ga = gamma ? __ldg(gamma + c) : 1.f;
-      const float bound = fabsf(ga * rs) * __ldg(g_amax) * (2.f + sqrtf((float)M)) * 1.001f;
-      if (bound > 0.f && bound < 3.0e38f) atomic_max_nonneg(amax, bound);
-    }
+  double sa, sb;
+  bn_fold_lanes(red_a, red_b, tx, sa, sb);
+  bn_finish_fwd(c, N, M, sa, sb, z_row0, gamma, beta, eps, momentum, running_mean, running_var, stats, affine);
+  if (amax) {
+    const float bound = bn_bound_fwd(c, M, gamma, beta, bound_mul);
+    if (bound > 0.f) atomic_max_nonneg(amax, bound);
   }
 }
 
@@ -173,75 +210,251 @@
   out[((long long)blockIdx.y * 2 + 1) * N + c] = t2;
 }
 
-__global__ void __launch_bounds__(256) bn_apply_planes_kernel(const float* __restrict__ z, long long M, int N, long long ldz,
-                                                              const float* __restrict__ affine, float drop_scale,
-                                                              unsigned thr, unsigned long long seed, unsigned long long offset,
-                                                              const unsigned long long* __restrict__ offset_dev,
-                                                              uint16_t* __restrict__ out, long long out_ld,
-                                                              long long plane_stride, unsigned char* __restrict__ mask,
-                                                              int ones_col, PlaneFmt fmt, FastDiv row_div) {
-  Philox rng{(unsigned)seed, (unsigned)(seed >> 32)};
-  if (offset_dev) offset += *offset_dev;
-  const float ps = fmt.scale();
-  const int n4 = N / 4;
-  const int n4o = (N + 7) / 8 * 2 + (ones_col ? 2 : 0);
-  const long long total = M * n4o;
-  const bool small = total < (1ll << 32);
-  for (long long i = (long long)blockIdx.x * blockDim.x + threadIdx.x; i < total; i += (long long)gridDim.x * blockDim.x) {
-    const long long r = small ? (long long)fastdiv((unsigned)i, row_div) : i / n4o;
-    const int c4 = (int)(i - r * n4o);
-    float4 v = make_float4(0.f, 0.f, 0.f, 0.f);
-    if (c4 < n4) {
-      const float4 zv = __ldg(reinterpret_cast<const float4*>(z + r * ldz) + c4);
-      const float4 sc = __ldg(reinterpret_cast<const float4*>(affine) + c4);
-      const float4 sh = __ldg(reinterpret_cast<const float4*>(affine + N) + c4);
-      const float4 y = make_float4(fmaf(zv.x, sc.x, sh.x), fmaf(zv.y, sc.y, sh.y), fmaf(zv.z, sc.z, sh.z), fmaf(zv.w, sc.w, sh.w));
-      uint4 q = make_uint4(0xffffffffu, 0xffffffffu, 0xffffffffu, 0xffffffffu);
-      if (thr) q = rng(offset + (unsigned long long)(r * n4 + c4));
-      uchar4 m;
-      m.x = (y.x > 0.f) && (q.x >= thr); m.y = (y.y > 0.f) && (q.y >= thr);
-      m.z = (y.z > 0.f) && (q.z >= thr); m.w = (y.w > 0.f) && (q.w >= thr);
-      *reinterpret_cast<uchar4*>(mask + r * (long long)N + c4 * 4) = m;
-      v = make_float4(m.x ? y.x * drop_scale : 0.f, m.y ? y.y * drop_scale : 0.f, m.z ? y.z * drop_scale : 0.f,
-                      m.w ? y.w * drop_scale : 0.f);
-    } else if (ones_col && c4 * 4 == ((N + 7) & ~7)) {
-      v.x = 1.f;
-    }
-    const float vv[4] = {v.x, v.y, v.z, v.w};
-    store_planes<4>(out + r * out_ld + c4 * 4, plane_stride, vv, fmt.format, ps);
-  }
-}
-
-__global__ void __launch_bounds__(256) bn_bwd_planes_kernel(const float* __restrict__ g, const float* __restrict__ z,
-                                                            long long M, int N, long long ldg, long long ldz,
-                                                            const float* __restrict__ stats, const float* __restrict__ sums,
-                                                            const float* __restrict__ gamma, uint16_t* __restrict__ out,
-                                                            long long out_ld, long long plane_stride, PlaneFmt fmt,
-                                                            FastDiv row_div) {
-  const float ps = fmt.scale();
-  const int n4 = N / 4;
-  const int n4o = (N + 7) / 8 * 2;
+constexpr int kSlabThreads = 1024;
+constexpr int kMaxSlab = 1024;
+
+struct BnSlabArgs {
+  const float* z;
+  const float* g;
+  long long M, ldz, ldg;
+  int N, slab, nblk;
+  int tile_f4;
+  const float* gamma;
+  const float* beta;
+  float eps, momentum;
+  float* running_mean;
+  float* running_var;
+  float* stats;
+  float* affine;
+  float* sums;
+  float bound_mul;
+  const float* g_amax;
+  float* bound_out;
+  float drop_scale;
+  unsigned thr;
+  unsigned long long seed, offset;
+  const unsigned long long* offset_dev;
+  unsigned char* mask;
+  int ones_col;
+  uint16_t* out;
+  long long out_ld, plane_stride;
+  PlaneFmt fmt;
+  float* partials;
+};
+
+__device__ __forceinline__ uint64_t l2_evict_last_policy() {
+  uint64_t pol;
+  asm volatile("createpolicy.fractional.L2::evict_last.b64 %0, 1.0;" : "=l"(pol));
+  return pol;
+}
+__device__ __forceinline__ void cp_async16(void* smem, const void* gmem, uint64_t pol) {
+  const unsigned s = (unsigned)__cvta_generic_to_shared(smem);
+  asm volatile("cp.async.cg.shared.global.L2::cache_hint [%0], [%1], 16, %2;" ::"r"(s), "l"(gmem), "l"(pol) : "memory");
+}
+__device__ __forceinline__ void cp_async_commit() { asm volatile("cp.async.commit_group;" ::: "memory"); }
+__device__ __forceinline__ void cp_async_wait1() { asm volatile("cp.async.wait_group 1;" ::: "memory"); }
+struct LdShared {
+  __device__ __forceinline__ float4 operator()(const float* p) const { return *reinterpret_cast<const float4*>(p); }
+};
+__device__ __forceinline__ void prefetch_l2(const void* p, unsigned bytes, uint64_t pol) {
+  asm volatile("cp.async.bulk.prefetch.L2.global.L2::cache_hint [%0], %1, %2;" ::"l"(p), "r"(bytes), "l"(pol) : "memory");
+}
+
+template <int MODE>
+__global__ void __launch_bounds__(kSlabThreads, 1) bn_slabs_kernel(const BnSlabArgs a) {
+  namespace cg = cooperative_groups;
+  cg::grid_group grid = cg::this_grid();
+  __shared__ double red_a[32][33], red_b[32][33];
+  __shared__ float4 s_par[MODE == 0 ? 2 : 5][kMaxSlab / 4];
+  __shared__ unsigned s_max[32];
+  extern __shared__ float4 s_tile[];
+  const int tid = threadIdx.x, lane = tid & 31, wid = tid >> 5;
+  const long long M = a.M;
+  const int N = a.N, n4 = N / 4;
+
+  float ps = 1.f;
+  {
+    unsigned bm = 0;
+    if (a.bound_out) {
+      for (int c = tid; c < N; c += kSlabThreads) {
+        const float b = MODE == 0 ? bn_bound_fwd(c, M, a.gamma, a.beta, a.bound_mul)
+                                  : bn_bound_bwd(c, N, M, a.gamma, a.stats, a.g_amax);
+        bm = max(bm, __float_as_uint(b));
+      }
+      bm = __reduce_max_sync(kFull, bm);
+      if (lane == 0) s_max[wid] = bm;
+      __syncthreads();
+      bm = __reduce_max_sync(kFull, s_max[lane]);
+      if (blockIdx.x == 0 && tid == 0 && bm) atomicMax(reinterpret_cast<unsigned*>(a.bound_out), bm);
+    }
+    if (a.fmt.format == kPlanesFp16x2) {
+      unsigned v = a.fmt.amax ? __float_as_uint(*reinterpret_cast<const volatile float*>(a.fmt.amax)) : 0u;
+      if (a.fmt.amax == a.bound_out) v = max(v, bm);
+      ps = plane_scale(__uint_as_float(v), a.fmt.max_exp);
+    }
+  }
+
+  const uint64_t keep = l2_evict_last_policy();
+  const long long gthreads = (long long)gridDim.x * kSlabThreads;
+  const long long gtid = (long long)blockIdx.x * kSlabThreads + tid;
+  const long long rows_per = (M + a.nblk - 1) / a.nblk;
+  const int n4o = (N + 7) / 8 * 2 + (MODE == 0 && a.ones_col ? 2 : 0);
   const float inv_m = 1.0f / (float)M;
-  const long long total = M * n4o;
-  const bool small = total < (1ll << 32);
-  for (long long i = (long long)blockIdx.x * blockDim.x + threadIdx.x; i < total; i += (long long)gridDim.x * blockDim.x) {
-    const long long r = small ? (long long)fastdiv((unsigned)i, row_div) : i / n4o;
-    const int c4 = (int)(i - r * n4o);
-    float4 v = make_float4(0.f, 0.f, 0.f, 0.f);
-    if (c4 < n4) {
-      const float4 gv = __ldg(reinterpret_cast<const float4*>(g + r * ldg) + c4);
-      const float4 zv = __ldg(reinterpret_cast<const float4*>(z + r * ldz) + c4);
-      const float4 mu = __ldg(reinterpret_cast<const float4*>(stats) + c4);
-      const float4 rs = __ldg(reinterpret_cast<const float4*>(stats + N) + c4);
-      const float4 db = __ldg(reinterpret_cast<const float4*>(sums) + c4);
-      const float4 dg = __ldg(reinterpret_cast<const float4*>(sums + N) + c4);
-      const float4 ga = gamma ? __ldg(reinterpret_cast<const float4*>(gamma) + c4) : make_float4(1.f, 1.f, 1.f, 1.f);
+  unsigned long long offset = a.offset;
+  if (MODE == 0 && a.offset_dev) offset += *a.offset_dev;
+  const Philox rng{(unsigned)a.seed, (unsigned)(a.seed >> 32)};
+
+  for (int c0 = 0; c0 < N; c0 += a.slab) {
+    const int w = min(a.slab, N - c0), w4 = w / 4, c40 = c0 / 4;
+
+    if (a.tile_f4) {
+      const int nmine = (a.nblk - (int)blockIdx.x + (int)gridDim.x - 1) / (int)gridDim.x;
+      auto issue = [&](int t) {
+        const long long r0 = rows_per * (blockIdx.x + (long long)t * gridDim.x);
+        const int rows = (int)(r0 < M ? (r0 + rows_per < M ? rows_per : M - r0) : 0);
+        float4* buf = s_tile + (t & 1) * a.tile_f4;
+        const int per = rows * w4;
+#pragma unroll 1
+        for (int mtx = 0; mtx <= MODE; ++mtx) {
+          const float* src = (mtx ? a.g + r0 * a.ldg : a.z + r0 * a.ldz) + c0;
+          const long long ld = mtx ? a.ldg : a.ldz;
+          float4* dst = buf + mtx * (rows_per * w4);
+          for (int e = tid; e < per; e += kSlabThreads) {
+            const int row = e / w4, j = e - row * w4;
+            cp_async16(dst + e, src + row * ld + 4 * j, keep);
+          }
+        }
+        cp_async_commit();
+      };
+      if (nmine > 0) issue(0);
+      for (int t = 0; t < nmine; ++t) {
+        if (t + 1 < nmine) issue(t + 1);
+        else cp_async_commit();
+        cp_async_wait1();
+        __syncthreads();
+        const int b = blockIdx.x + t * gridDim.x;
+        const long long r0 = rows_per * b;
+        const long long r1 = r0 + rows_per < M ? r0 + rows_per : M;
+        for (int j = tid; j < w4; j += kSlabThreads) {
+          const int c4 = c40 + j;
+          float4 k, rs = make_float4(1.f, 1.f, 1.f, 1.f);
+          if (MODE == 0) {
+            k = __ldg(reinterpret_cast<const float4*>(a.z) + c4);
+          } else {
+            k = __ldg(reinterpret_cast<const float4*>(a.stats) + c4);
+            rs = __ldg(reinterpret_cast<const float4*>(a.stats + N) + c4);
+          }
+          const float* tz = reinterpret_cast<const float*>(s_tile + (t & 1) * a.tile_f4);
+          const float* tg = tz + rows_per * w;
+          float4 sa, sb;
+          bn_row_sums<MODE>(tz, tg, w, w, 0, r1 > r0 ? r1 - r0 : 0, j, k, rs, sa, sb, LdShared{});
+          float* pa = a.partials + ((long long)b * 2) * N;
+          __stcg(reinterpret_cast<float4*>(pa) + c4, sa);
+          __stcg(reinterpret_cast<float4*>(pa + N) + c4, sb);
+        }
+        __syncthreads();
+      }
+    } else {
+      for (long long r = gtid; r < M; r += gthreads) {
+        prefetch_l2(a.z + r * a.ldz + c0, (unsigned)w * 4u, keep);
+        if (MODE == 1) prefetch_l2(a.g + r * a.ldg + c0, (unsigned)w * 4u, keep);
+      }
+      const int items = a.nblk * w4;
+      for (int i = (wid * gridDim.x + blockIdx.x) * 32 + lane; i - lane < items; i += gridDim.x * kSlabThreads) {
+        if (i >= items) continue;
+        const int b = i / w4, c4 = c40 + (i - b * w4);
+        const long long r0 = rows_per * b;
+        const long long r1 = r0 + rows_per < M ? r0 + rows_per : M;
+        float4 k, rs = make_float4(1.f, 1.f, 1.f, 1.f);
+        if (MODE == 0) {
+          k = __ldg(reinterpret_cast<const float4*>(a.z) + c4);
+        } else {
+          k = __ldg(reinterpret_cast<const float4*>(a.stats) + c4);
+          rs = __ldg(reinterpret_cast<const float4*>(a.stats + N) + c4);
+        }
+        float4 sa, sb;
+        bn_row_sums<MODE, LdKeep, MODE == 0 ? 8 : 2>(a.z, a.g, a.ldz, a.ldg, r0, r1, c4, k, rs, sa, sb, LdKeep{keep});
+        float* pa = a.partials + ((long long)b * 2) * N;
+        __stcg(reinterpret_cast<float4*>(pa) + c4, sa);
+        __stcg(reinterpret_cast<float4*>(pa + N) + c4, sb);
+      }
+    }
+    grid.sync();
+
+    for (int grp = blockIdx.x; grp * 32 < w; grp += gridDim.x) {
+      const int c = c0 + grp * 32 + lane;
+      const bool ok = c < c0 + w;
+      double la = 0.0, lb = 0.0;
+      if (ok) bn_fold_lane(a.partials, a.nblk, N, c, wid, la, lb);
+      red_a[wid][lane] = la;
+      red_b[wid][lane] = lb;
+      __syncthreads();
+      if (wid == 0 && ok) {
+        double sa, sb;
+        bn_fold_lanes(red_a, red_b, lane, sa, sb);
+        if (MODE == 0) {
+          bn_finish_fwd(c, N, M, sa, sb, a.z, a.gamma, a.beta, a.eps, a.momentum, a.running_mean, a.running_var, a.stats,
+                        a.affine);
+        } else {
+          a.sums[c] = (float)sa;
+          a.sums[N + c] = (float)sb;
+        }
+      }
+      __syncthreads();
+    }
+    grid.sync();
+
+    for (int j = tid; j < w4; j += kSlabThreads) {
+      const int c4 = c40 + j;
+      if (MODE == 0) {
+        s_par[0][j] = __ldcg(reinterpret_cast<const float4*>(a.affine) + c4);
+        s_par[1][j] = __ldcg(reinterpret_cast<const float4*>(a.affine + N) + c4);
+      } else {
+        s_par[0][j] = __ldg(reinterpret_cast<const float4*>(a.stats) + c4);
+        s_par[1][j] = __ldg(reinterpret_cast<const float4*>(a.stats + N) + c4);
+        s_par[2][j] = __ldcg(reinterpret_cast<const float4*>(a.sums) + c4);
+        s_par[3][j] = __ldcg(reinterpret_cast<const float4*>(a.sums + N) + c4);
+        s_par[4][j] = a.gamma ? __ldg(reinterpret_cast<const float4*>(a.gamma) + c4) : make_float4(1.f, 1.f, 1.f, 1.f);
+      }
+    }
+    __syncthreads();
+    const int cw4 = w4 + (c0 + w >= N ? n4o - n4 : 0);
+    const long long total = M * cw4;
+    const bool small = total < (1ll << 32);
+    const FastDiv row_div = make_fastdiv((unsigned long long)cw4);
+    for (long long i = gtid; i < total; i += gthreads) {
+      const long long r = small ? (long long)fastdiv((unsigned)i, row_div) : i / cw4;
+      const int j = (int)(i - r * cw4);
+      const int c4 = j < w4 ? c40 + j : n4 + (j - w4);
+      float4 v = make_float4(0.f, 0.f, 0.f, 0.f);
+      if (j < w4) {
+        const float4 zv = __ldlu(reinterpret_cast<const float4*>(a.z + r * a.ldz) + c4);
+        if (MODE == 0) {
+          const float4 sc = s_par[0][j], sh = s_par[1][j];
+          const float4 y = make_float4(fmaf(zv.x, sc.x, sh.x), fmaf(zv.y, sc.y, sh.y), fmaf(zv.z, sc.z, sh.z),
+                                       fmaf(zv.w, sc.w, sh.w));
+          uint4 q = make_uint4(0xffffffffu, 0xffffffffu, 0xffffffffu, 0xffffffffu);
+          if (a.thr) q = rng(offset + (unsigned long long)(r * n4 + c4));
+          uchar4 m;
+          m.x = (y.x > 0.f) && (q.x >= a.thr); m.y = (y.y > 0.f) && (q.y >= a.thr);
+          m.z = (y.z > 0.f) && (q.z >= a.thr); m.w = (y.w > 0.f) && (q.w >= a.thr);
+          *reinterpret_cast<uchar4*>(a.mask + r * (long long)N + c4 * 4) = m;
+          v = make_float4(m.x ? y.x * a.drop_scale : 0.f, m.y ? y.y * a.drop_scale : 0.f,
+                          m.z ? y.z * a.drop_scale : 0.f, m.w ? y.w * a.drop_scale : 0.f);
+        } else {
+          const float4 gv = __ldlu(reinterpret_cast<const float4*>(a.g + r * a.ldg) + c4);
+          const float4 mu = s_par[0][j], rs = s_par[1][j], db = s_par[2][j], dg = s_par[3][j], ga = s_par[4][j];
 #define RSB_BN_BWD(f) (ga.f * rs.f * (gv.f - db.f * inv_m - (zv.f - mu.f) * rs.f * dg.f * inv_m))
-      v = make_float4(RSB_BN_BWD(x), RSB_BN_BWD(y), RSB_BN_BWD(z), RSB_BN_BWD(w));
+          v = make_float4(RSB_BN_BWD(x), RSB_BN_BWD(y), RSB_BN_BWD(z), RSB_BN_BWD(w));
 #undef RSB_BN_BWD
-    }
-    const float vv[4] = {v.x, v.y, v.z, v.w};
-    store_planes<4>(out + r * out_ld + c4 * 4, plane_stride, vv, fmt.format, ps);
+        }
+      } else if (MODE == 0 && a.ones_col && c4 * 4 == ((N + 7) & ~7)) {
+        v.x = 1.f;
+      }
+      const float vv[4] = {v.x, v.y, v.z, v.w};
+      store_planes<4>(a.out + r * a.out_ld + c4 * 4, a.plane_stride, vv, a.fmt.format, ps);
+    }
+    __syncthreads();
   }
 }
 
@@ -250,6 +463,70 @@
   const long long need = (M + 31) / 32;
   if (b > need) b = need;
   return b < 1 ? 1 : (int)b;
+}
+
+static long long l2_bytes() {
+  static long long cached[64] = {0};
+  int dev = 0;
+  if (cudaGetDevice(&dev) != cudaSuccess || dev < 0 || dev >= 64) return 0;
+  if (cached[dev] == 0) {
+    int n = 0;
+    if (cudaDeviceGetAttribute(&n, cudaDevAttrL2CacheSize, dev) != cudaSuccess || n <= 0) n = 0;
+    cached[dev] = n;
+  }
+  return cached[dev];
+}
+
+static int bn_slab_cols(long long M, int N, int bytes_per_elem) {
+  long long w = l2_bytes() / 3 / (M * bytes_per_elem) / 16 * 16;
+  if (w < 16) w = 16;
+  if (w > kMaxSlab) w = kMaxSlab;
+  return N <= w ? N : (int)w;
+}
+
+constexpr int kTileSmem = 160 * 1024;
+
+template <int MODE>
+static int bn_slabs_grid(long long work) {
+  static int cached[64] = {0};
+  int dev = 0;
+  if (cudaGetDevice(&dev) != cudaSuccess || dev < 0 || dev >= 64) return 0;
+  if (cached[dev] == 0) {
+    int occ = 0;
+    if (cudaFuncSetAttribute(bn_slabs_kernel<MODE>, cudaFuncAttributeMaxDynamicSharedMemorySize, kTileSmem) != cudaSuccess ||
+        cudaOccupancyMaxActiveBlocksPerMultiprocessor(&occ, bn_slabs_kernel<MODE>, kSlabThreads, kTileSmem) != cudaSuccess)
+      return 0;
+    cached[dev] = occ * sm_count();
+  }
+  long long g = (work + kSlabThreads - 1) / kSlabThreads;
+  if (g > cached[dev]) g = cached[dev];
+  return g < 1 ? 1 : (int)g;
+}
+
+template <int MODE>
+static int launch_bn_slabs(BnSlabArgs& args, long long work, cudaStream_t st) {
+  const int grid = bn_slabs_grid<MODE>(work);
+  if (grid <= 0) return RSB_ERR_UNSUPPORTED;
+  const long long rows_per = (args.M + args.nblk - 1) / args.nblk;
+  const long long tile_f4 = rows_per * (args.slab / 4) * (MODE + 1);
+  args.tile_f4 = 2 * tile_f4 * 16 <= kTileSmem ? (int)tile_f4 : 0;
+  cudaLaunchConfig_t cfg = {};
+  cfg.gridDim = dim3((unsigned)grid);
+  cfg.blockDim = dim3(kSlabThreads);
+  cfg.dynamicSmemBytes = (size_t)args.tile_f4 * 2 * 16;
+  cfg.stream = st;
+  cudaLaunchAttribute attr[1];
+  attr[0].id = cudaLaunchAttributeCooperative;
+  attr[0].val.cooperative = 1;
+  cfg.attrs = attr;
+  cfg.numAttrs = 1;
+  const cudaError_t e = cudaLaunchKernelEx(&cfg, bn_slabs_kernel<MODE>, args);
+  if (e != cudaSuccess) {
+    (void)cudaGetLastError();
+    return (int)e;
+  }
+  note_launch(1);
+  return RSB_OK;
 }
 
 }
@@ -273,10 +550,10 @@
   float* partials = reinterpret_cast<float*>((reinterpret_cast<uintptr_t>(workspace) + 255) / 256 * 256);
   cudaStream_t st = reinterpret_cast<cudaStream_t>(stream);
   const int nblk = bn_blocks(M);
-  bn_slab_sums_kernel<0><<<nblk, kBnThreads, 0, st>>>(z, nullptr, M, N, ldz, 0, nullptr, nullptr, partials);
+  bn_slab_sums_kernel<<<nblk, kBnThreads, 0, st>>>(z, M, N, ldz, partials);
   RSB_CHECK_LAUNCH();
-  bn_finalize_kernel<0><<<(N + 31) / 32, 1024, 0, st>>>(partials, nblk, N, M, z, gamma, beta, eps, momentum, running_mean,
-                                                     running_var, stats, affine, nullptr, bound_mul, nullptr, act_amax);
+  bn_finalize_kernel<<<(N + 31) / 32, 1024, 0, st>>>(partials, nblk, N, M, z, gamma, beta, eps, momentum, running_mean,
+                                                  running_var, stats, affine, bound_mul, act_amax);
   RSB_CHECK_LAUNCH();
   note_launch(2);
   return RSB_OK;
@@ -297,33 +574,58 @@
   if (slices > groups) slices = (int)groups;
   bn_parts_fold_kernel<<<dim3((N + 31) / 32, slices), 1024, 0, st>>>(parts, groups, N, M, sl);
   RSB_CHECK_LAUNCH();
-  bn_finalize_kernel<0><<<(N + 31) / 32, 1024, 0, st>>>(sl, slices, N, M, parts + 2 * (long long)N, gamma, beta, eps, momentum,
-                                                     running_mean, running_var, stats, affine, nullptr, bound_mul, nullptr, act_amax);
+  bn_finalize_kernel<<<(N + 31) / 32, 1024, 0, st>>>(sl, slices, N, M, parts + 2 * (long long)N, gamma, beta, eps, momentum,
+                                                  running_mean, running_var, stats, affine, bound_mul, act_amax);
   RSB_CHECK_LAUNCH();
   note_launch(2);
   return RSB_OK;
 }
 
-extern "C" RSB_API int rsb_bn_relu_dropout_planes(const float* z, int64_t M, int32_t N, int64_t ldz, const float* affine, float p,
-                                                  uint64_t seed, uint64_t offset, const uint64_t* offset_dev, int32_t ones_col,
-                                                  void* out_planes, int64_t out_ld, int64_t plane_stride, uint8_t* mask,
-                                                  const rsb_planes_format* fmt, void* stream) {
-  if (!z || !affine || !out_planes || !mask || M < 0 || N <= 0 || p < 0.f || p >= 1.f || !plane_fmt_ok(fmt)) return RSB_ERR_BAD_ARG;
-  if (M == 0) return RSB_OK;
-  if (N % 4 || ldz % 4 || out_ld % 8 || plane_stride % 8 || out_ld < ((N + 7) / 8) * 8 + (ones_col ? 8 : 0) || !aligned16(z) ||
-      !aligned16(affine) || !aligned16(out_planes) || (reinterpret_cast<uintptr_t>(mask) & 3u))
+extern "C" RSB_API int rsb_bn_train_fwd_planes(const float* z, int64_t M, int32_t N, int64_t ldz, const float* gamma,
+                                               const float* beta, float eps, float momentum, float* running_mean,
+                                               float* running_var, float* stats, float* affine, float bound_mul,
+                                               float* act_amax, float p, uint64_t seed, uint64_t offset,
+                                               const uint64_t* offset_dev, int32_t ones_col, void* out_planes, int64_t out_ld,
+                                               int64_t plane_stride, uint8_t* mask, const rsb_planes_format* fmt,
+                                               void* workspace, int64_t workspace_bytes, void* stream) {
+  if (!z || !stats || !affine || !out_planes || !mask || M <= 0 || N <= 0 || p < 0.f || p >= 1.f || !plane_fmt_ok(fmt))
+    return RSB_ERR_BAD_ARG;
+  if (N % 4 || ldz % 4 || out_ld % 8 || plane_stride % 8 || out_ld < ((N + 7) / 8) * 8 + (ones_col ? 8 : 0) ||
+      !aligned16(z) || !aligned16(stats) || !aligned16(affine) || (gamma && !aligned16(gamma)) ||
+      (beta && !aligned16(beta)) || !aligned16(out_planes) || (reinterpret_cast<uintptr_t>(mask) & 3u))
     return RSB_ERR_UNSUPPORTED;
-  const long long total = M * ((N + 7) / 8 * 2 + (ones_col ? 2 : 0));
-  long long blocks = (total + 255) / 256;
-  const long long cap = (long long)sm_count() * 16;
-  if (blocks > cap) blocks = cap;
-  bn_apply_planes_kernel<<<(unsigned)blocks, 256, 0, reinterpret_cast<cudaStream_t>(stream)>>>(
-      z, M, N, ldz, affine, 1.0f / (1.0f - p), (unsigned)(p * 4294967296.0), seed, offset,
-      reinterpret_cast<const unsigned long long*>(offset_dev), reinterpret_cast<uint16_t*>(out_planes), out_ld, plane_stride,
-      mask, ones_col, plane_fmt(fmt), make_fastdiv((unsigned long long)((N + 7) / 8 * 2 + (ones_col ? 2 : 0))));
-  RSB_CHECK_LAUNCH();
-  note_launch(1);
-  return RSB_OK;
+  if (!workspace || workspace_bytes < rsb_bn_workspace_bytes(M, N)) return RSB_ERR_WORKSPACE;
+  BnSlabArgs a = {};
+  a.z = z;
+  a.M = M;
+  a.ldz = ldz;
+  a.N = N;
+  a.slab = bn_slab_cols(M, N, 4);
+  a.nblk = bn_blocks(M);
+  a.gamma = gamma;
+  a.beta = beta;
+  a.eps = eps;
+  a.momentum = momentum;
+  a.running_mean = running_mean;
+  a.running_var = running_var;
+  a.stats = stats;
+  a.affine = affine;
+  a.bound_mul = bound_mul;
+  a.bound_out = act_amax;
+  a.drop_scale = 1.0f / (1.0f - p);
+  a.thr = (unsigned)(p * 4294967296.0);
+  a.seed = seed;
+  a.offset = offset;
+  a.offset_dev = reinterpret_cast<const unsigned long long*>(offset_dev);
+  a.mask = mask;
+  a.ones_col = ones_col;
+  a.out = reinterpret_cast<uint16_t*>(out_planes);
+  a.out_ld = out_ld;
+  a.plane_stride = plane_stride;
+  a.fmt = plane_fmt(fmt);
+  a.partials = reinterpret_cast<float*>((reinterpret_cast<uintptr_t>(workspace) + 255) / 256 * 256);
+  const long long work = M * ((N + 7) / 8 * 2 + (ones_col ? 2 : 0));
+  return launch_bn_slabs<0>(a, work, reinterpret_cast<cudaStream_t>(stream));
 }
 
 extern "C" RSB_API int rsb_bn_train_bwd_planes(const float* g, const float* z, int64_t M, int32_t N, int64_t ldg, int64_t ldz,
@@ -336,23 +638,25 @@
       !aligned16(z) || !aligned16(stats) || !aligned16(sums) || !aligned16(out_planes) || (gamma && !aligned16(gamma)))
     return RSB_ERR_UNSUPPORTED;
   if (!workspace || workspace_bytes < rsb_bn_workspace_bytes(M, N)) return RSB_ERR_WORKSPACE;
-  float* partials = reinterpret_cast<float*>((reinterpret_cast<uintptr_t>(workspace) + 255) / 256 * 256);
-  cudaStream_t st = reinterpret_cast<cudaStream_t>(stream);
-  const int nblk = bn_blocks(M, 4);
   const bool h = fmt && fmt->format == kPlanesFp16x2;
-  bn_slab_sums_kernel<1><<<nblk, kBnThreads, 0, st>>>(z, g, M, N, ldz, ldg, stats, stats + N, partials);
-  RSB_CHECK_LAUNCH();
-  bn_finalize_kernel<1><<<(N + 31) / 32, 1024, 0, st>>>(partials, nblk, N, M, nullptr, gamma, nullptr, 0.f, 0.f, nullptr, nullptr,
-                                                     sums, nullptr, stats, 1.f, h ? g_amax : nullptr, h ? fmt->amax : nullptr);
-  RSB_CHECK_LAUNCH();
-  const long long total = M * ((N + 7) / 8 * 2);
-  long long blocks = (total + 255) / 256;
-  const long long cap = (long long)sm_count() * 16;
-  if (blocks > cap) blocks = cap;
-  bn_bwd_planes_kernel<<<(unsigned)blocks, 256, 0, st>>>(g, z, M, N, ldg, ldz, stats, sums, gamma,
-                                                         reinterpret_cast<uint16_t*>(out_planes), out_ld, plane_stride,
-                                                         plane_fmt(fmt), make_fastdiv((unsigned long long)((N + 7) / 8 * 2)));
-  RSB_CHECK_LAUNCH();
-  note_launch(3);
-  return RSB_OK;
-}
+  BnSlabArgs a = {};
+  a.z = z;
+  a.g = g;
+  a.M = M;
+  a.ldz = ldz;
+  a.ldg = ldg;
+  a.N = N;
+  a.slab = bn_slab_cols(M, N, 8);
+  a.nblk = bn_blocks(M, 4);
+  a.gamma = gamma;
+  a.stats = const_cast<float*>(stats);
+  a.sums = sums;
+  a.g_amax = h ? g_amax : nullptr;
+  a.bound_out = h ? fmt->amax : nullptr;
+  a.out = reinterpret_cast<uint16_t*>(out_planes);
+  a.out_ld = out_ld;
+  a.plane_stride = plane_stride;
+  a.fmt = plane_fmt(fmt);
+  a.partials = reinterpret_cast<float*>((reinterpret_cast<uintptr_t>(workspace) + 255) / 256 * 256);
+  return launch_bn_slabs<1>(a, M * ((N + 7) / 8 * 2), reinterpret_cast<cudaStream_t>(stream));
+}
diff --git a/recsys-benchmark_b200/linalg.py b/recsys-benchmark_b200/linalg.py
--- a/recsys-benchmark_b200/linalg.py
+++ b/recsys-benchmark_b200/linalg.py
@@ -479,20 +479,23 @@
         for i in range(n_layers):
             bn = bns[i]
             act_amax = amaxs[i + 1] if (amaxs is not None and i < n_layers - 1) else None
-            z, st, affine = P.gemm_bn_stats(planes[-1], weight_planes(ws[i], fmt=planes[-1].fmt), bs[i], gammas[i],
-                                            betas[i], bn.eps, bn.momentum,
-                                            bn.running_mean if bn.track_running_stats else None,
-                                            bn.running_var if bn.track_running_stats else None,
-                                            act_amax=act_amax, bound_mul=1.0 / (1.0 - ps[i]), in_epilogue=BN_STATS_IN_GEMM)
+            wp = weight_planes(ws[i], fmt=planes[-1].fmt)
+            rm = bn.running_mean if bn.track_running_stats else None
+            rv = bn.running_var if bn.track_running_stats else None
+            if i < n_layers - 1:
+                xp = planes[-1]
+                z = P.gemm(xp, wp, xp.rows, wp.rows, wp.cols, bias=bs[i], split_k=1)
+                seed, off = _dropout_stream(z.numel())
+                yp, mask, st, affine = P.bn_train_fwd_planes(z, gammas[i], betas[i], bn.eps, bn.momentum, rm, rv, ps[i],
+                                                             seed, off, _DROPOUT_DEV_COUNTER, ones_col=True, fmt=fmt,
+                                                             amax=act_amax)
+                planes.append(yp)
+            else:
+                z, st, affine = P.gemm_bn_stats(planes[-1], wp, bs[i], gammas[i], betas[i], bn.eps, bn.momentum, rm, rv,
+                                                in_epilogue=BN_STATS_IN_GEMM)
+                y, mask, out = _relu_dropout_dot_fwd(z, ps[i], w_out.reshape(-1), b_out, affine)
             if bn.track_running_stats and bn.num_batches_tracked is not None:
                 bn.num_batches_tracked.add_(1)
-            if i < n_layers - 1:
-                seed, off = _dropout_stream(z.numel())
-                yp, mask = P.bn_relu_dropout_planes(z, affine, ps[i], seed, off, _DROPOUT_DEV_COUNTER, ones_col=True,
-                                                    fmt=fmt, amax=act_amax)
-                planes.append(yp)
-            else:
-                y, mask, out = _relu_dropout_dot_fwd(z, ps[i], w_out.reshape(-1), b_out, affine)
             masks.append(mask)
             zs.append(z)
             stats.append(st)
diff --git a/recsys-benchmark_b200/planes.py b/recsys-benchmark_b200/planes.py
--- a/recsys-benchmark_b200/planes.py
+++ b/recsys-benchmark_b200/planes.py
@@ -237,20 +237,26 @@
     return z, stats, affine
 
 
-def bn_relu_dropout_planes(z: torch.Tensor, affine: torch.Tensor, p: float, seed: int, offset: int,
-                           offset_dev: Optional[torch.Tensor] = None, ones_col: bool = True, fmt: int = BF16X3,
-                           amax: Optional[torch.Tensor] = None):
-    lib = L.load()
-    m, n = z.shape
+def bn_train_fwd_planes(z: torch.Tensor, gamma: Optional[torch.Tensor], beta: Optional[torch.Tensor], eps: float,
+                        momentum: float, running_mean: Optional[torch.Tensor], running_var: Optional[torch.Tensor],
+                        p: float, seed: int, offset: int, offset_dev: Optional[torch.Tensor] = None, ones_col: bool = True,
+                        fmt: int = BF16X3, amax: Optional[torch.Tensor] = None):
+    lib = L.load()
+    m, n = z.shape
+    dev = z.device
     assert fmt == BF16X3 or amax is not None
-    yp = alloc(m, n, z.device, ones_col, fmt, amax)
+    yp = alloc(m, n, dev, ones_col, fmt, amax)
     pf = yp.format()
-    mask = torch.empty(m, n, dtype=torch.uint8, device=z.device)
-    RF._call("bn_relu_dropout_planes", lib.rsb_bn_relu_dropout_planes, L.ptr(z), m, n, z.stride(0), L.ptr(affine), float(p),
-             seed & 0xFFFFFFFFFFFFFFFF, offset & 0xFFFFFFFFFFFFFFFF, L.ptr(offset_dev), int(ones_col), L.ptr(yp.data), yp.ld,
-             yp.data.stride(0), L.ptr(mask), C.byref(pf), L.stream_ptr(z.device),
-             nbytes=m * n * 5 + yp.data.shape[0] * m * yp.ld * 2)
-    return yp, mask
+    mask = torch.empty(m, n, dtype=torch.uint8, device=dev)
+    stats = torch.empty(2 * n, dtype=torch.float32, device=dev)
+    affine = torch.empty(2 * n, dtype=torch.float32, device=dev)
+    ws = RF._ws(lib.rsb_bn_workspace_bytes(m, n), dev)
+    RF._call("bn_fwd_planes", lib.rsb_bn_train_fwd_planes, L.ptr(z), m, n, z.stride(0), L.ptr(gamma), L.ptr(beta),
+             float(eps), float(momentum), L.ptr(running_mean), L.ptr(running_var), L.ptr(stats), L.ptr(affine),
+             float(1.0 / (1.0 - p)), L.ptr(amax), float(p), seed & 0xFFFFFFFFFFFFFFFF, offset & 0xFFFFFFFFFFFFFFFF,
+             L.ptr(offset_dev), int(ones_col), L.ptr(yp.data), yp.ld, yp.data.stride(0), L.ptr(mask), C.byref(pf),
+             L.ptr(ws), ws.numel(), L.stream_ptr(dev), nbytes=m * n * 5 + yp.data.shape[0] * m * yp.ld * 2)
+    return yp, mask, stats, affine
 
 
 def bn_train_bwd_planes(g: torch.Tensor, z: torch.Tensor, stats: torch.Tensor, gamma: Optional[torch.Tensor],
```

Result: slower. 23.30 million, median of 6 (-12.9%).
